# maria-korosteleva/Garment-Pattern-Estimation

Measured on AMD Instinct MI355X. Metric: garments/sec (fwd+bwd) at N=2048 pts, batch 32 per GPU, higher is better.
Workload: dtype f16x3 (fp16 MFMA x3 per product, fp32 accumulate); 1 GPU; BASELINE cfg 2 (cfg 3 per GPU): GarmentFullPattern3D, EdgeConv encoder + LSTM decoders, N=2048, batch 32/GPU, k=16; fp32 storage, fp32-grade arithmetic: edge-GEMM products as 3 fp16 MFMAs on tensor-normalised two-term splits, fp32 accumulate (parity-grade: the exact mode's test bars); global_batch=32, parallelism=dp1, math_mode=f16x3, loss_epoch=0, reserved_cus=0, launch=eager (one Python call per launch), side_stream=True, step=fwd + ComposedPatternLoss + bwd + fused Adam (flat arena)

## Files before the change

garment-pattern-estimation_amd/csrc/gpe_edge_dispatch.h:

```cpp
#pragma once
#include "gpe_rowgemm.h"

#define GPE_EDGE_LAUNCHED 1
#define GPE_EDGE_NOT_MINE 0

static inline bool gpe_edge_width_ok(int c) { return c > 96 && c <= 208; }
static inline int gpe_edge_chunks(int c) { return c <= 160 ? 10 : 13; }
enum { GPE_EDGE_F2 = 0, GPE_EDGE_F3 = 1, GPE_EDGE_B3 = 2, GPE_EDGE_B2 = 3 };
constexpr int gpe_edge_kind(int amode, int emode)
{
    return emode == E_EDGE_FWD ? (amode == A_GATHER ? GPE_EDGE_F2 : GPE_EDGE_F3) : (emode == E_BWD_INPLACE ? GPE_EDGE_B3 : GPE_EDGE_B2);
}
static inline bool gpe_edge_on_menu(const RgParams& p, int amode, int emode)
{
    if (!gpe_edge_width_ok(p.N) || !gpe_edge_width_ok(p.K)) return false;
    if (emode != E_EDGE_FWD && (p.N & 3)) return false;
    if (amode == A_GATHER && (p.K & 3)) return false;
    return !(amode == A_DENSE && (p.a.inner > 0 || (p.a.stride_outer & 3) || p.a.stride_outer < ((p.K + 3) & ~3) || (((uintptr_t)p.a.base) & 15)));
}

int gpe_edge_pseudo_kq(int k);
size_t gpe_edge_pseudo_bytes(long npts, int k, int Cmax);
bool gpe_edge_retile(const RgParams& p_in, int amode, int emode, int stats_nblk, RgParams& p, GpeFold& fold);
int gpe_edge_finish(int rc, const RgParams& p, const GpeFold& fold, hipStream_t s);

int gpe_edge_pc(const RgParams& p, int amode, int emode, int NT, int KCH, int bf16x3, int stats_nblk, hipStream_t s);
int gpe_edge_sr(const RgParams& p, int amode, int emode, int NT, int KCH, int stats_nblk, hipStream_t s);
int gpe_edge_bf16x6(const RgParams& p, int amode, int emode, int NT, int KCH, int stats_nblk, hipStream_t s);
int gpe_edge_f16x3_scales(RgParams& p, long npts, int amode, int emode, int KCH, hipStream_t s);
int gpe_edge_f16x3(const RgParams& p, int amode, int emode, int NT, int KCH, int stats_nblk, hipStream_t s);
int gpe_edge_w8(const RgParams& p, int amode, int emode, int NT, int KCH, int stats_nblk, hipStream_t s);

template <int A, int E> struct GpeEdgeMode { static constexpr int amode = A, emode = E, kind = gpe_edge_kind(A, E); };
template <int AQ_, int BQ_, int KCH_> struct GpeEdgeTile { static constexpr int AQ = AQ_, BQ = BQ_, KCH = KCH_, NT = 4 * AQ_ + BQ_; };

template <class F> static inline int gpe_edge_for_mode(int amode, int emode, F&& f)
{
    if (amode == A_GATHER && emode == E_EDGE_FWD) return f(GpeEdgeMode<A_GATHER, E_EDGE_FWD>{});
    if (amode == A_DENSE && emode == E_EDGE_FWD) return f(GpeEdgeMode<A_DENSE, E_EDGE_FWD>{});
    if (amode == A_DENSE && emode == E_BWD_INPLACE) return f(GpeEdgeMode<A_DENSE, E_BWD_INPLACE>{});
    if (amode == A_DENSE && emode == E_BWD_GATHER) return f(GpeEdgeMode<A_DENSE, E_BWD_GATHER>{});
    return GPE_EINVAL;
}
template <class F> static inline int gpe_edge_for_tile(int NT, int KCH, F&& f)
{
    if (NT == 13 && KCH == 13) return f(GpeEdgeTile<3, 1, 13>{});
    if (NT == 13 && KCH == 10) return f(GpeEdgeTile<3, 1, 10>{});
    if (NT == 10 && KCH == 13) return f(GpeEdgeTile<2, 2, 13>{});
    if (NT == 10 && KCH == 10) return f(GpeEdgeTile<2, 2, 10>{});
    return GPE_EDGE_NOT_MINE;
}
template <class MENU, class F> static inline int gpe_edge_select(int amode, int emode, int NT, int KCH, F&& f)
{
    return gpe_edge_for_mode(amode, emode, [&](auto m) {
        return gpe_edge_for_tile(NT, KCH, [&](auto t) -> int {
            if constexpr (MENU::has(decltype(m)::amode, decltype(m)::emode, decltype(t)::NT, decltype(t)::KCH)) return f(m, t);
            else return GPE_EDGE_NOT_MINE;
        });
    });
}

#define GPE_EDGE_LDS_CAP (160 * 1024)
#define GPE_EDGE_LDS_CAP_STATIC (160 * 1024 - 64)
template <auto KERNEL, int BLOCK, int LDS_CAP> static int gpe_edge_launch(const RgParams& p, int stats_nblk, size_t lds, hipStream_t s)
{
    GPE_ENSURE_MAX_LDS_N(KERNEL, LDS_CAP);
    int gx = gpe_num_cus();
    if (gx > p.num_tiles) gx = p.num_tiles;
    if (stats_nblk > 0 && gx > stats_nblk) gx = stats_nblk;
    hipLaunchKernelGGL(KERNEL, dim3(gx), dim3(BLOCK), lds, s, p, stats_nblk);
    GPE_CHECK_LAUNCH();
    return GPE_EDGE_LAUNCHED;
}
```

garment-pattern-estimation_amd/csrc/gpe_edge_dispatch.hip:

```cpp
#include "gpe_edge_dispatch.h"

static int g_eg_math = 0;
void gpe_edgegemm_set_math(int m) { g_eg_math = m; }

int gpe_edge_pseudo_kq(int k)
{
    int best = 0;
    for (int kq = RG_PB; kq >= RG_PB / RG_NPW; --kq)
        if (k % kq == 0 && (RG_PB / kq) * kq > (best ? (RG_PB / best) * best : 0)) best = kq;
    return best;
}

size_t gpe_edge_pseudo_bytes(long npts, int k, int Cmax)
{
    const int kq = k <= RG_PB ? 0 : gpe_edge_pseudo_kq(k);
    if (!kq) return 0;
    const size_t nps = (size_t)npts * (k / kq), ld = (size_t)((Cmax + 3) & ~3);
    return nps * ld * (2 * sizeof(float) + 2) + 256;
}

static bool edge_pseudo_setup(RgParams& p, bool per_point, int emode, GpeFold& fd)
{
    fd = GpeFold{};
    fd.f = 1;
    if (p.k <= RG_PB) return true;
    if (!per_point) { p.k = 4; return true; }
    const long npts = p.M / p.k;
    const int kq = gpe_edge_pseudo_kq(p.k);
    if (!kq || npts * (p.k / kq) >= (1L << 31) || (p.oldagg & 3) || (p.lddp & 3)) return false;
    fd.f = p.k / kq; fd.kq = kq; fd.npts = npts;
    const long nps = npts * fd.f;
    const bool want_agg = emode == E_EDGE_FWD && p.agg, want_dp = emode == E_BWD_GATHER;
    const size_t agg_f = want_agg ? (size_t)nps * p.oldagg : 0, dp_f = want_dp ? (size_t)nps * p.lddp : 0;
    const size_t bytes = (2 * agg_f + dp_f) * sizeof(float) + 2 * agg_f + 256;
    char* ws = (bytes > 256 && bytes <= p.ws.pseudo_bytes) ? p.ws.pseudo : nullptr;
    if (bytes > 256 && !ws) return false;
    if (want_agg) {
        fd.mx = p.mx; fd.mn = p.mn; fd.amx = p.oamx; fd.amn = p.oamn;
        p.mx = (float*)ws; p.mn = p.mx + agg_f;
        p.oamx = (uint8_t*)(p.mn + agg_f); p.oamn = p.oamx + agg_f;
    }
    if (want_dp) { fd.dp = p.dP; p.dP = (float*)ws; }
    p.k = kq;
    p.pmagic = (unsigned)(((1ull << 32) + fd.f - 1) / fd.f);
    return true;
}

bool gpe_edge_retile(const RgParams& p_in, int amode, int emode, int stats_nblk, RgParams& p, GpeFold& fold)
{
    p = p_in;
    const bool per_point = amode == A_GATHER || emode == E_BWD_GATHER || (emode == E_EDGE_FWD && p.agg);
    if (!edge_pseudo_setup(p, per_point, emode, fold)) return false;
    const int npw = RG_PB / p.k;
    if (per_point && npw > RG_NPW) return false;
    p.R = 4 * npw * p.k;
    p.num_tiles = gpe_cdiv(p.M, p.R);
    p.pin_tpc = 0;
    if ((amode == A_GATHER || emode == E_BWD_GATHER) && p.pin_clouds > 0 && gpe_pin_clouds(p.pin_clouds) &&
        p.pin_clouds % GPE_NXCD == 0) {
        const long rows_per_cloud = p.M / p.pin_clouds;
        const int gx = gpe_num_cus();
        if (rows_per_cloud % p.R == 0 && gx % GPE_NXCD == 0 && gx <= p.num_tiles &&
            (stats_nblk <= 0 || gx <= stats_nblk) && rows_per_cloud / p.R >= gx / GPE_NXCD)
            p.pin_tpc = (int)(rows_per_cloud / p.R);
    }
    return true;
}

int gpe_edge_finish(int rc, const RgParams& p, const GpeFold& fold, hipStream_t s)
{
    if (rc != GPE_EDGE_LAUNCHED) return rc;
    rc = gpe_edge_pseudo_fold(p, fold, s);
    return rc == GPE_OK ? GPE_EDGE_LAUNCHED : rc;
}

int gpe_edgegemm_try(const RgParams& p, int amode, int emode, int stats_nblk, hipStream_t s)
{
    const int math = g_eg_math;
    const bool f16_only = p.out_half || p.lz_g;
    if (!gpe_edge_on_menu(p, amode, emode)) return f16_only ? GPE_EINVAL : GPE_EDGE_NOT_MINE;
    const int NT = gpe_edge_chunks(p.N), KCH = gpe_edge_chunks(p.K);

    RgParams t;
    GpeFold fold;
    const bool tiled = math != 1 && p.k >= 1 && gpe_edge_retile(p, amode, emode, stats_nblk, t, fold);
    int rc;

    if (math == 2 && tiled) {
        rc = gpe_edge_finish(gpe_edge_bf16x6(t, amode, emode, NT, KCH, stats_nblk, s), t, fold, s);
        if (rc != GPE_EDGE_NOT_MINE) return rc;
    }
    if (math == 3 && tiled && p.ws.h3 && p.M >= gpe_h3_min_rows() && !(amode == A_GATHER && !p.user_amax_a && (p.H & 3))) {
        RgParams q = t;
        rc = gpe_edge_f16x3_scales(q, p.M / p.k, amode, emode, KCH, s);
        if (rc != GPE_OK) return rc;
        rc = gpe_edge_w8(q, amode, emode, NT, KCH, stats_nblk, s);
        if (rc == GPE_EDGE_NOT_MINE) rc = gpe_edge_f16x3(q, amode, emode, NT, KCH, stats_nblk, s);
        rc = gpe_edge_finish(rc, q, fold, s);
        if (rc == GPE_EDGE_LAUNCHED && q.amax_out && p.tracked) *p.tracked = 1;
        if (rc != GPE_EDGE_NOT_MINE) return rc;
    }
    if (f16_only) return GPE_EINVAL;

    if (math != 1 && tiled && !(p.dbg & 64)) {
        rc = gpe_edge_finish(gpe_edge_sr(t, amode, emode, NT, KCH, stats_nblk, s), t, fold, s);
        if (rc != GPE_EDGE_NOT_MINE) return rc;
    }
    if (p.R <= 64 && p.k <= 64)
        return gpe_edge_pc(p, amode, emode, NT, KCH, math == 1, stats_nblk, s);
    return GPE_EDGE_NOT_MINE;
}
```

garment-pattern-estimation_amd/csrc/gpe_edgegemm_w8.hip:

```cpp
#include "gpe_edgegemm_w8_kernel.h"

int gpe_w8_select_k5(const RgParams& p, int amode, int emode, int NT, int KCH, int stats_nblk, hipStream_t s);
int gpe_w8_select_k4(const RgParams& p, int amode, int emode, int NT, int KCH, int stats_nblk, hipStream_t s);

static int w8_enabled(int kind)
{
    static int tab[4] = {-1, 0, 0, 0};
    if (tab[0] < 0) {
        const char* e = gpe_dbg_env_str("GPE_W8");
        for (int i = 3; i >= 0; --i) {
            int v = 1;
            if (e && strlen(e) == 4) v = e[i] != '0';
            else if (e && strlen(e) == 1) v = e[0] != '0';
            tab[i] = v;
        }
    }
    return tab[kind];
}

int gpe_edge_w8(const RgParams& p, int amode, int emode, int NT, int KCH, int stats_nblk, hipStream_t s)
{
    if (!((p.k == 16 && p.R == 64 && !p.pmagic) || (p.k == 5 && p.R == 60 && !p.pmagic) || (p.k == 4 && p.R == 64)) || p.M % p.k)
        return GPE_EDGE_NOT_MINE;
    const int kbytes = 2 * ((p.K + 3) & ~3);
    if (kbytes < (KCH == 13 ? 384 : 256)) return GPE_EDGE_NOT_MINE;
    if (p.out_half && !(p.k == 16 && emode == E_EDGE_FWD && amode == A_DENSE && p.agg)) return GPE_EINVAL;
    if (p.lz_g && !(p.k == 16 && emode == E_BWD_INPLACE && amode == A_DENSE)) return GPE_EINVAL;
    if (!w8_enabled(gpe_edge_kind(amode, emode))) return GPE_EDGE_NOT_MINE;
    return p.k == 16 ? w8_select<16>(p, amode, emode, NT, KCH, stats_nblk, s)
           : p.k == 5 ? gpe_w8_select_k5(p, amode, emode, NT, KCH, stats_nblk, s)
                      : gpe_w8_select_k4(p, amode, emode, NT, KCH, stats_nblk, s);
}
```

garment-pattern-estimation_amd/csrc/gpe_edgegemm_w8_kernel.h:

```cpp
#pragma once
#include "gpe_edgegemm_split_kernel.h"
#include <type_traits>

#ifndef W8_SLOT_FENCE
#define W8_SLOT_FENCE 1
#endif
#ifndef W8_B2_SC1
#define W8_B2_SC1 1
#endif
#ifndef W8_BUFSTORE
#define W8_BUFSTORE 11
#endif
__device__ __forceinline__ void w8_pin4(float4& v) { asm volatile("" : "+v"(v.x), "+v"(v.y), "+v"(v.z), "+v"(v.w)); }

template <int NT, int KCH, int AMODE, int EMODE, int AGGT, bool LAZY, int KK = 16>
__global__ __launch_bounds__(512) void gpe_edgegemm_w8_kernel(RgParams p, int stats_nblk)
{
    using SP = SplitF16x2;
    static_assert(KK == 16 || KK == 5 || KK == 4, "neighbourhood sizes with a compile-time row schedule");
    static_assert(!LAZY || KK == 16, "lazy dz3 needs one point per wave");
    constexpr int NPW = 16 / KK;
    constexpr int RW = NPW * KK;
    constexpr int TR = 4 * RW;
    static_assert(NT == 13 || (NT == 10 && KCH == 13), "shapes of the shipped edge MLPs");
    static_assert(KCH == 13 || KCH == 10, "K = 200 / 150");
    static_assert(!LAZY || (AMODE == A_DENSE && EMODE == E_BWD_INPLACE), "lazy dz3: in-place backward");
    static_assert(EMODE != E_BWD_INPLACE || (W8_BUFSTORE & 4) == 0, "the in-place backward loads the rows it overwrites through plain "
                  "pointers: its stores must be plain too (buffer and global accesses are disjoint memory to the compiler)");
    constexpr bool FWD = EMODE == E_EDGE_FWD;
    constexpr bool TRACK = FWD && AGGT != 0;
    constexpr bool OUTH = FWD && AGGT == 2;
    constexpr bool GATHER_ACT = EMODE == E_BWD_GATHER;
    constexpr int KS = (KCH + 1) / 2;
    constexpr bool KTAIL = (KCH & 1) != 0;
    constexpr bool PAIRS = NT == 13;
    constexpr int SL2 = PAIRS ? (KS + 1) / 2 : (KS + 3) / 4;
    constexpr int PPITCH = 16 * x6_pchunks(KCH);
    constexpr int PLANE = RG_BM * PPITCH;
    constexpr int AWORDS = (2 * PLANE) / 4;
    constexpr int LDC = 16 * NT + 4;
    constexpr int NSLOT = 4 * KS;
    constexpr int SPP = (KCH == 13) ? 6 : 4;
    constexpr int NLS = PAIRS ? KS - 1 : 0;
    constexpr int NSCR = PAIRS ? 4 + NLS : 6;
    static_assert(NSCR <= 2 * SPP, "partials do not fit the row");
    constexpr int C0 = (NSLOT >= 28) ? 8 : 6;
    constexpr int I1 = C0 + 4;
    constexpr int C1 = (NSLOT >= 28) ? 22 : 16;
    constexpr int EP0 = NSLOT - 16;
    constexpr int RING = (GATHER_ACT && NPW > 1) ? 6 : 8;

    extern __shared__ __align__(16) float smem[];
    __shared__ unsigned amax_sh[4];
    __shared__ int flag_sh[4];
    float* const Abuf0 = smem;
    float* const Abuf1 = smem + AWORDS;
    float* const Cs = smem + 2 * AWORDS;

    const int tid = threadIdx.x, lane = tid & 63;
    const int wave = __builtin_amdgcn_readfirstlane(tid >> 6);
    const int role = wave >> 2, pt = wave & 3;
    const int j = lane & 15, g = lane >> 4;
    const int g_tail = (g >= 2) ? (g & 1) : g;
    const int rb = RW * pt;
    const int c = lane << 2;
    const bool n_on = c < p.N;
    const int ck = (c < p.K) ? c : ((p.K - 1) & ~3);
    const int cn = n_on ? c : ((p.N - 1) & ~3);

    int rot, sec_tile, sec_slot;
    bool sec_direct, last_on = false, last_direct = false;
    int last_slot = 0;
    if constexpr (PAIRS) {
        rot = role ? pt + SL2 : pt;
        if (rot >= KS) rot -= KS;
        sec_tile = 8 + pt; sec_direct = role == 0; sec_slot = pt;
        last_on = role == 0 || rot >= 4;
        last_direct = wave == 0;
        last_slot = 4 + (role == 0 ? pt - 1 : rot - 1);
    } else {
        rot = 2 * pt;
        sec_tile = 8 + role; sec_direct = pt == 0; sec_slot = 3 * role + pt - 1;
    }

    for (int e = tid; e < 2 * AWORDS; e += 512) smem[e] = 0.f;
    if (tid < 4) flag_sh[tid] = 0;

    float sA, sW, invA, invW;
    SP::scale_of(p.h3_amax_a[0], sA, invA);
    SP::scale_of(p.h3_amax_w[0], sW, invW);

    gpe_u32x4 wP[2][KS], sP[2][SL2], tP[2];
    {
        auto load_frag = [&](int col, int sl) -> X6Frag<SP> {
            const int cc = (col < p.Npad) ? col : p.Npad - 1;
            const int kc = 2 * sl + (g >> 1);
            const bool on = col < p.Npad && kc < KCH;
            const int kcc = kc < KCH ? kc : KCH - 1;
            float4 f0 = ld4(p.wp + (((long)(kcc * 4 + 2 * (g & 1))) * p.Npad + cc) * 4);
            float4 f1 = ld4(p.wp + (((long)(kcc * 4 + 2 * (g & 1) + 1)) * p.Npad + cc) * 4);
            f0 = x6_scale4(f0, sW); f1 = x6_scale4(f1, sW);
            const float4 z = make_float4(0.f, 0.f, 0.f, 0.f);
            return x6_split8<SP>(on ? f0 : z, on ? f1 : z);
        };
#pragma unroll
        for (int i = 0; i < KS; ++i) {
            const int sl = (rot + i >= KS) ? rot + i - KS : rot + i;
            const X6Frag<SP> f = load_frag(16 * wave + j, sl);
            wP[0][i] = f.pl[0]; wP[1][i] = f.pl[1];
        }
#pragma unroll
        for (int i = 0; i < SL2; ++i) {
            const int sl = (rot + i >= KS) ? rot + i - KS : rot + i;
            const bool real = PAIRS ? (role == 0 || i < KS - SL2) : (rot + i < KS);
            const X6Frag<SP> f = load_frag(real ? 16 * sec_tile + j : p.Npad, sl);
            sP[0][i] = f.pl[0]; sP[1][i] = f.pl[1];
        }
        {
            const X6Frag<SP> f = load_frag((PAIRS && last_on) ? 16 * 12 + j : p.Npad, rot);
            tP[0] = f.pl[0]; tP[1] = f.pl[1];
        }
    }

    GpeTileSeq sq = gpe_tile_seq(p.pin_tpc, p.rev, p.pin_clouds, p.num_tiles);

    int vz;
    asm volatile("v_mov_b32 %0, 0" : "=v"(vz));
    int rbl = rb;
#define W8_REFRESH_SCALARS()                                   \
    {                                                          \
        int sz_;                                               \
        asm volatile("s_mov_b32 %0, 0" : "=s"(sz_));           \
        rbl = rb + sz_;                                        \
    }
    auto load_jgv = [&](int tile) -> int {
        const long row0 = (long)tile * TR;
        const int rv = (int)((p.M - row0 < TR) ? (p.M - row0) : TR);
        int r = rbl + ((lane < RW) ? lane : RW - 1);
        r = (r < rv - 1) ? r : rv - 1;
        return p.jg[row0 + r];
    };
    auto prow = [&](long x) -> long { return (KK == 4 && p.pmagic) ? (long)__umulhi((unsigned)x, p.pmagic) : x; };
    auto scr = [&](int row, int s) -> int { return ((s >= SPP ? PLANE + (s - SPP) * 64 : s * 64) + row * PPITCH) >> 2; };

    auto body = [&](auto role_tag) {
        constexpr int ROLE = decltype(role_tag)::value;
        const float4 zero4 = make_float4(0.f, 0.f, 0.f, 0.f);

        float4 v[8];
        constexpr int NPB = NPW > 1 ? 2 : 1;
        float4 pvs[NPB];
#pragma unroll
        for (int q = 0; q < NPB; ++q) pvs[q] = zero4;
        int s_rv = 0, jgv_a = 0, jgv_b = 0;
        float lzs[4] = {0.f, 0.f, 0.f, 0.f}, lznc[4] = {0.f, 0.f, 0.f, 0.f}, lznk[4] = {0.f, 0.f, 0.f, 0.f};
        int lz_sel[4] = {0, 0, 0, 0};
        float lz_won[4] = {0.f, 0.f, 0.f, 0.f};
        float4 lz_gq = zero4;
        uchar4 lz_sx = make_uchar4(0, 0, 0, 0), lz_sn = make_uchar4(0, 0, 0, 0);
        if constexpr (ROLE == 0 && LAZY) {
#pragma unroll
            for (int t = 0; t < 4; ++t) {
                if (ck + t < p.K) {
                    const float k2 = p.lz_coef[2 * p.K + ck + t];
                    lzs[t] = p.lz_coef[ck + t] * sA;
                    lznc[t] = __builtin_fmaf(p.lz_coef[3 * p.K + ck + t], k2, -p.lz_coef[p.K + ck + t]) * sA;
                    lznk[t] = -k2 * sA;
                }
            }
        }
        double stS[4] = {0, 0, 0, 0}, stQ[4] = {0, 0, 0, 0};
        float4 bias4 = zero4, cs4 = zero4, c14 = zero4, k24 = zero4;
        if constexpr (ROLE == 1) {
            {
                if constexpr (FWD) {
                    if (p.bias) {
                        bias4.x = p.bias[cn];
                        if (cn + 1 < p.N) bias4.y = p.bias[cn + 1];
                        if (cn + 2 < p.N) bias4.z = p.bias[cn + 2];
                        if (cn + 3 < p.N) bias4.w = p.bias[cn + 3];
                    }
                } else {
                    cs4 = ld4(p.coef_out + cn); c14 = ld4(p.coef_out + p.N + cn);
                    cs4 = x6_scale4(cs4, invW * invA);
                    k24 = ld4(p.coef_out + 2 * p.N + cn);
                    const float4 mu4 = ld4(p.coef_out + 3 * p.N + cn);
                    c14 = make_float4(__builtin_fmaf(mu4.x, k24.x, -c14.x), __builtin_fmaf(mu4.y, k24.y, -c14.y),
                                      __builtin_fmaf(mu4.z, k24.z, -c14.z), __builtin_fmaf(mu4.w, k24.w, -c14.w));
                    k24 = make_float4(-k24.x, -k24.y, -k24.z, -k24.w);
                }
            }
        }
        const float invAW = invA * invW;
        float amax_run = 0.f;
        float s32[4] = {0.f, 0.f, 0.f, 0.f}, q32[4] = {0.f, 0.f, 0.f, 0.f};
        float vmx[4], vmn[4];
        int imx[4], imn[4];
#pragma unroll
        for (int t = 0; t < 4; ++t) { vmx[t] = -INFINITY; vmn[t] = INFINITY; imx[t] = 0; imn[t] = 0; }
        float4 dp = zero4;
        float4 act[(ROLE == 1 && !FWD) ? RING : 1];
        constexpr int NPE = NPW > 3 ? 2 : NPW;
        float4 pve[NPE];
        long e_ptl = 0;
#pragma unroll
        for (int q = 0; q < NPE; ++q) pve[q] = zero4;
        long e_row0 = 0, e_pt = 0; int e_rv = 0;
        bool epi_on = false;
        __amdgpu_buffer_rsrc_t orsrc = __builtin_amdgcn_make_buffer_rsrc(p.out, 0, 0, 0x00020000);
        float amax_t = 0.f;
        int jgv_e = 0, jgv_cur = 0;

        auto issue_stage_loads = [&](int tile_s, int h) {
            const long row0 = (long)tile_s * TR;
            s_rv = (int)((p.M - row0 < TR) ? (p.M - row0) : TR);
            const int last = s_rv - 1;
            const long pt0 = (long)tile_s * (4 * NPW) + pt * NPW, ptl = (long)tile_s * (4 * NPW) + last / KK;
            const long ptc = pt0 < ptl ? pt0 : ptl;
            if (h == 0) {
                if constexpr (LAZY) {
                    const float* gr = p.lz_g + ptc * p.lz_ldg + ck;
                    const int rem = p.K - 1 - ck;
                    lz_gq = make_float4(gr[0], gr[rem < 1 ? rem : 1], gr[rem < 2 ? rem : 2], gr[rem < 3 ? rem : 3]);
                    lz_sx = *reinterpret_cast<const uchar4*>(p.lz_amx + ptc * p.lz_ldagg + ck);
                    lz_sn = *reinterpret_cast<const uchar4*>(p.lz_amn + ptc * p.lz_ldagg + ck);
                }
            }
            if constexpr (AMODE == A_GATHER) {
                const int pb = (8 * h) / KK;
#pragma unroll
                for (int q = 0; q < NPB; ++q) {
                    const long pg = pt0 + ((pb + q < NPW) ? pb + q : NPW - 1);
                    pvs[q] = ld4(p.pq + (prow(pg < ptl ? pg : ptl) + vz) * p.ldpq + ck);
                }
            }
#pragma unroll
            for (int uu = 0; uu < 8; ++uu) {
                const int u = (8 * h + uu < RW) ? 8 * h + uu : RW - 1;
                int r = rbl + u;
                r = (r < last) ? r : last;
                if constexpr (AMODE == A_GATHER) {
                    const int jj = __builtin_amdgcn_ds_bpermute(u << 2, jgv_a);
                    v[uu] = ld4(p.pq + (long)jj * p.ldpq + p.H + ck);
                } else if constexpr (LAZY) {
                    const uint2 hq = *reinterpret_cast<const uint2*>(reinterpret_cast<const _Float16*>(p.a.base) + (row0 + r) * p.a.stride_outer + ck);
                    v[uu].x = __uint_as_float(hq.x); v[uu].y = __uint_as_float(hq.y);
                } else
                    v[uu] = ld4(p.a.base + (row0 + r) * p.a.stride_outer + ck);
            }
        };
        auto commit_row = [&](float* An, int u) {
            if (u >= RW) return;
            const int r = rbl + u;
            float4 o = v[u & 7];
            if constexpr (AMODE == A_GATHER) {
                const float4 pv = pvs[u / KK - (8 * (u / 8)) / KK];
                o.x = fmaxf(o.x + pv.x, 0.f); o.y = fmaxf(o.y + pv.y, 0.f);
                o.z = fmaxf(o.z + pv.z, 0.f); o.w = fmaxf(o.w + pv.w, 0.f);
            }
            if constexpr (LAZY) {
                const gpe_f32x2 a01 = __builtin_convertvector(__builtin_bit_cast(gpe_f16x2, __float_as_uint(o.x)), gpe_f32x2);
                const gpe_f32x2 a23 = __builtin_convertvector(__builtin_bit_cast(gpe_f16x2, __float_as_uint(o.y)), gpe_f32x2);
                const float av[4] = {a01[0], a01[1], a23[0], a23[1]};
                if (u == 0) {
                    const float gq[4] = {lz_gq.x, lz_gq.y, lz_gq.z, lz_gq.w};
                    const int sx[4] = {lz_sx.x, lz_sx.y, lz_sx.z, lz_sx.w}, sn[4] = {lz_sn.x, lz_sn.y, lz_sn.z, lz_sn.w};
#pragma unroll
                    for (int t = 0; t < 4; ++t) {
                        lz_sel[t] = (lzs[t] >= 0.f) ? sx[t] : sn[t];
                        lz_won[t] = __builtin_fmaf(lzs[t], gq[t], lznc[t]);
                    }
                }
                float dz[4];
#pragma unroll
                for (int t = 0; t < 4; ++t) {
                    const float base = (lz_sel[t] == u) ? lz_won[t] : lznc[t];
                    dz[t] = (av[t] > 0.f) ? __builtin_fmaf(lznk[t], av[t], base) : 0.f;
                }
                o = make_float4(dz[0], dz[1], dz[2], dz[3]);
            }
            if (r >= s_rv) o = zero4;
            unsigned q0[2], q1[2];
            const float sc = LAZY ? 1.f : sA;
            SP::split2(o.x * sc, o.y * sc, q0);
            SP::split2(o.z * sc, o.w * sc, q1);
            char* row = reinterpret_cast<char*>(An) + r * PPITCH + 2 * ck;
            *reinterpret_cast<uint2*>(row) = make_uint2(q0[0], q1[0]);
            *reinterpret_cast<uint2*>(row + PLANE) = make_uint2(q0[1], q1[1]);
        };
        auto wait_folded = [&](int want) {
            int spins = 0;
            while (__hip_atomic_load(&flag_sh[pt], __ATOMIC_ACQUIRE, __HIP_MEMORY_SCOPE_WORKGROUP) < want) {
                __builtin_amdgcn_s_sleep(1);
                if (++spins > (1 << 22)) __builtin_trap();
            }
        };

        auto issue_act_load = [&](int u, int tile_e, int jv) {
            if constexpr (ROLE == 1 && !FWD) {
                const long row0 = (long)tile_e * TR;
                const int rv = (int)((p.M - row0 < TR) ? (p.M - row0) : TR);
                if (u >= RW) u = RW - 1;
                int r = rbl + u;
                r = (r < rv - 1) ? r : rv - 1;
                if constexpr (EMODE == E_BWD_INPLACE) act[u % RING] = ld4(p.out + (row0 + r) * p.ldo + cn);
                else {
                    const int jj = __builtin_amdgcn_ds_bpermute(u << 2, jv);
                    act[u % RING] = ld4(p.pq + (long)jj * p.ldpq + p.H + cn);
                }
            }
        };
        auto begin_epi = [&](int tile_e, bool on) {
            e_row0 = (long)tile_e * TR;
            e_pt = (long)tile_e * (4 * NPW) + pt * NPW;
            e_rv = (int)((p.M - e_row0 < TR) ? (p.M - e_row0) : TR);
            epi_on = on && rbl < e_rv;
            constexpr int ES = OUTH ? 2 : 4;
            orsrc = __builtin_amdgcn_make_buffer_rsrc(reinterpret_cast<char*>(p.out) + e_row0 * p.ldo * ES, 0, RG_BM * p.ldo * ES, 0x00020000);
#pragma unroll
            for (int t = 0; t < 4; ++t) { s32[t] = 0.f; q32[t] = 0.f; vmx[t] = -INFINITY; vmn[t] = INFINITY; imx[t] = 0; imn[t] = 0; }
            dp = zero4;
            amax_t = 0.f;
            if constexpr (GATHER_ACT) {
                const long ptl = (long)tile_e * (4 * NPW) + (e_rv - 1) / KK;
                if constexpr (NPW > NPE) e_ptl = ptl;
#pragma unroll
                for (int q = 0; q < NPE; ++q) pve[q] = ld4(p.pq + (prow(e_pt + q < ptl ? e_pt + q : ptl) + vz) * p.ldpq + cn);
            }
        };
        auto epi_row = [&](int u, float4 z) {
            if (u >= RW) return;
            if constexpr (GATHER_ACT && NPW > NPE) {
                if (u % KK == 0 && u / KK >= 1) {
                    const int q = u / KK;
                    w8_pin4(pve[q % NPE]);
                    if (q + 1 < NPW) {
                        const long pg = e_pt + q + 1;
                        pve[(q + 1) % NPE] = ld4(p.pq + (prow(pg < e_ptl ? pg : e_ptl) + vz) * p.ldpq + cn);
                    }
                }
            }
            w8_pin4(z);
            if constexpr (!FWD) w8_pin4(act[u % RING]);
            if (!epi_on) return;
            const int r = rbl + u;
            if constexpr (KK != 16) {
                if (r >= e_rv) return;
            }
            if constexpr (FWD) {
                const float vv[4] = {fmaxf(__builtin_fmaf(z.x, invAW, bias4.x), 0.f), fmaxf(__builtin_fmaf(z.y, invAW, bias4.y), 0.f),
                                     fmaxf(__builtin_fmaf(z.z, invAW, bias4.z), 0.f), fmaxf(__builtin_fmaf(z.w, invAW, bias4.w), 0.f)};
                if constexpr (!TRACK) amax_t = fmaxf(fmaxf(amax_t, fmaxf(vv[0], vv[1])), fmaxf(vv[2], vv[3]));
                if constexpr (OUTH) {
                    const gpe_f32x2 v01 = {fminf(vv[0], 65504.f), fminf(vv[1], 65504.f)}, v23 = {fminf(vv[2], 65504.f), fminf(vv[3], 65504.f)};
                    const gpe_u32x2 hq = {__builtin_bit_cast(unsigned, __builtin_convertvector(v01, gpe_f16x2)),
                                         __builtin_bit_cast(unsigned, __builtin_convertvector(v23, gpe_f16x2))};
                    if constexpr ((W8_BUFSTORE & 2) != 0)
                        __builtin_amdgcn_raw_buffer_store_b64(hq, orsrc, cn * 2, r * p.ldo * 2, 0);
                    else
                        *reinterpret_cast<uint2*>(reinterpret_cast<_Float16*>(p.out) + (e_row0 + r) * p.ldo + cn) = make_uint2(hq[0], hq[1]);
                } else {
                    const gpe_u32x4 oq = {__float_as_uint(vv[0]), __float_as_uint(vv[1]), __float_as_uint(vv[2]), __float_as_uint(vv[3])};
                    if constexpr ((W8_BUFSTORE & (AMODE == A_GATHER ? 1 : 2)) != 0)
                        __builtin_amdgcn_raw_buffer_store_b128(oq, orsrc, cn * 4, r * p.ldo * 4, AMODE == A_GATHER ? 16 : 0);
                    else
                        st4(p.out + (e_row0 + r) * p.ldo + cn, make_float4(vv[0], vv[1], vv[2], vv[3]));
                }
#pragma unroll
                for (int t = 0; t < 4; ++t) {
                    s32[t] += vv[t];
                    q32[t] = __builtin_fmaf(vv[t], vv[t], q32[t]);
                    if constexpr (TRACK) {
                        if (vv[t] > vmx[t]) { vmx[t] = vv[t]; imx[t] = u % KK; }
                        if (vv[t] < vmn[t]) { vmn[t] = vv[t]; imn[t] = u % KK; }
                    }
                }
            } else {
                float4 av = act[u % RING];
                if constexpr (GATHER_ACT) {
                    const float4 pv = pve[(u / KK) % NPE];
                    av.x = fmaxf(av.x + pv.x, 0.f); av.y = fmaxf(av.y + pv.y, 0.f);
                    av.z = fmaxf(av.z + pv.z, 0.f); av.w = fmaxf(av.w + pv.w, 0.f);
                }
                float4 o;
                o.x = (av.x > 0.f) ? __builtin_fmaf(z.x, cs4.x, __builtin_fmaf(k24.x, av.x, c14.x)) : 0.f;
                o.y = (av.y > 0.f) ? __builtin_fmaf(z.y, cs4.y, __builtin_fmaf(k24.y, av.y, c14.y)) : 0.f;
                o.z = (av.z > 0.f) ? __builtin_fmaf(z.z, cs4.z, __builtin_fmaf(k24.z, av.z, c14.z)) : 0.f;
                o.w = (av.w > 0.f) ? __builtin_fmaf(z.w, cs4.w, __builtin_fmaf(k24.w, av.w, c14.w)) : 0.f;
                const gpe_u32x4 oq = {__float_as_uint(o.x), __float_as_uint(o.y), __float_as_uint(o.z), __float_as_uint(o.w)};
                if constexpr ((W8_BUFSTORE & (EMODE == E_BWD_INPLACE ? 4 : 8)) != 0)
                    __builtin_amdgcn_raw_buffer_store_b128(oq, orsrc, cn * 4, r * p.ldo * 4, (GATHER_ACT && W8_B2_SC1) ? 16 : 0);
                else
                    st4(p.out + (e_row0 + r) * p.ldo + cn, o);
                if constexpr (EMODE == E_BWD_INPLACE)
                    amax_t = fmaxf(fmaxf(amax_t, fmaxf(fabsf(o.x), fabsf(o.y))), fmaxf(fabsf(o.z), fabsf(o.w)));
                dp.x += o.x; dp.y += o.y; dp.z += o.z; dp.w += o.w;
            }
            if (u % KK == KK - 1) {
                if constexpr (TRACK) amax_t = fmaxf(amax_t, fmaxf(fmaxf(vmx[0], vmx[1]), fmaxf(vmx[2], vmx[3])));
                {
                    const long gpt = e_pt + u / KK;
                    if constexpr (TRACK) {
                        const long o = gpt * p.oldagg + cn;
                        st4(p.mx + o, make_float4(vmx[0], vmx[1], vmx[2], vmx[3]));
                        st4(p.mn + o, make_float4(vmn[0], vmn[1], vmn[2], vmn[3]));
                        *reinterpret_cast<uchar4*>(p.oamx + o) = make_uchar4(imx[0], imx[1], imx[2], imx[3]);
                        *reinterpret_cast<uchar4*>(p.oamn + o) = make_uchar4(imn[0], imn[1], imn[2], imn[3]);
                    }
                    if constexpr (GATHER_ACT) st4(p.dP + gpt * p.lddp + cn, dp);
                }
                amax_run = fmaxf(amax_run, amax_t);
                if constexpr (FWD) {
#pragma unroll
                    for (int t = 0; t < 4; ++t) { stS[t] += (double)s32[t]; stQ[t] += (double)q32[t]; }
                }
                if constexpr (NPW > 1) {
#pragma unroll
                    for (int t = 0; t < 4; ++t) { vmx[t] = -INFINITY; vmn[t] = INFINITY; imx[t] = 0; imn[t] = 0; s32[t] = 0.f; q32[t] = 0.f; }
                    dp = zero4;
                }
            }
        };

        int tile = gpe_seq_tile(sq);
        gpe_seq_advance(sq);
        int next = gpe_seq_tile(sq);
        gpe_seq_advance(sq);
        int next2 = gpe_seq_tile(sq);
        if constexpr (ROLE == 0) {
            if (tile < p.num_tiles) {
                if constexpr (AMODE == A_GATHER) jgv_a = load_jgv(tile);
#pragma unroll
                for (int h = 0; h < 2; ++h) {
                    issue_stage_loads(tile, h);
#pragma unroll
                    for (int uu = 0; uu < 8; ++uu) commit_row(Abuf0, 8 * h + uu);
                }
                if constexpr (AMODE == A_GATHER) jgv_b = load_jgv(next < p.num_tiles ? next : tile);
            }
        }
        __syncthreads();

        int buf = 0, prev = -1, iter = 0;
        for (; tile < p.num_tiles; tile = next, next = next2, gpe_seq_advance(sq), next2 = gpe_seq_tile(sq)) {
            W8_REFRESH_SCALARS()
            const float* As = buf ? Abuf1 : Abuf0;
            float* An = buf ? Abuf0 : Abuf1;
            const bool do_epi = prev >= 0;
            const bool do_stage = next < p.num_tiles;
            const int tile_s = do_stage ? next : tile;
            const int tile_e = do_epi ? prev : tile;

            f32x4 acc[4], accS[4], accT[4];
#pragma unroll
            for (int mt = 0; mt < 4; ++mt) {
                acc[mt] = (f32x4){0.f, 0.f, 0.f, 0.f}; accS[mt] = acc[mt]; accT[mt] = acc[mt];
            }
            X6Frag<SP> nf;
            auto read_frag = [&](int i, int mt) {
                const int slr = (rot + i >= KS) ? rot + i - KS : rot + i;
                const int ge = (KTAIL && slr == KS - 1) ? g_tail : g;
                const char* src = reinterpret_cast<const char*>(As) + (16 * mt + j) * PPITCH + 16 * (4 * slr + ge);
                nf.pl[0] = *reinterpret_cast<const gpe_u32x4*>(src);
                nf.pl[1] = *reinterpret_cast<const gpe_u32x4*>(src + PLANE);
            };
            float4 zq = zero4;
            read_frag(0, 0);

#pragma unroll
            for (int i = 0; i < KS; ++i) {
#pragma unroll
                for (int mt = 0; mt < 4; ++mt) {
                    const int q = 4 * i + mt;
                    const X6Frag<SP> af = nf;
                    if (q + 1 < NSLOT) read_frag((q + 1) >> 2, (q + 1) & 3);
                    if constexpr (ROLE == 0) {
                        if (q == 0) {
                            if constexpr (AMODE == A_GATHER) {
                                jgv_a = jgv_b;
                                jgv_b = load_jgv(next2 < p.num_tiles ? next2 : tile);
                            }
                            issue_stage_loads(tile_s, 0);
                        }
                        if (q == C0) wait_folded(iter);
                        if (q >= C0 && q < C0 + 4) { commit_row(An, 2 * (q - C0)); commit_row(An, 2 * (q - C0) + 1); }
                        if (q == I1) issue_stage_loads(tile_s, 1);
                        if (q >= C1 && q < C1 + 4) { commit_row(An, 8 + 2 * (q - C1)); commit_row(An, 9 + 2 * (q - C1)); }
                    } else {
                        if (q == 0) {
                            begin_epi(tile_e, do_epi);
                            if constexpr (GATHER_ACT) { jgv_cur = jgv_e; jgv_e = load_jgv(tile); }
                        }
                        if (q >= EP0 && q - EP0 < RW) {
                            epi_row(q - EP0, zq);
                            if (q - EP0 + RING < RW) issue_act_load(q - EP0 + RING, tile_e, jgv_cur);
                            else issue_act_load((q - EP0) % RING, tile, jgv_e);
                        }
                        if (q + 1 >= EP0 && q + 1 < NSLOT) {
                            const int rr = rbl + ((q + 1 - EP0 < RW) ? q + 1 - EP0 : RW - 1);
                            zq = ld4(&Cs[rr * LDC + cn]);
                        }
                    }
                    acc[mt] = SP::mfma(af.pl[1], wP[0][i], acc[mt]);
                    if (i < SL2) accS[mt] = SP::mfma(af.pl[1], sP[0][i], accS[mt]);
                    if (PAIRS && i == 0) accT[mt] = SP::mfma(af.pl[1], tP[0], accT[mt]);
                    acc[mt] = SP::mfma(af.pl[0], wP[1][i], acc[mt]);
                    if (i < SL2) accS[mt] = SP::mfma(af.pl[0], sP[1][i], accS[mt]);
                    if (PAIRS && i == 0) accT[mt] = SP::mfma(af.pl[0], tP[1], accT[mt]);
                    acc[mt] = SP::mfma(af.pl[0], wP[0][i], acc[mt]);
                    if (i < SL2) accS[mt] = SP::mfma(af.pl[0], sP[0][i], accS[mt]);
                    if (PAIRS && i == 0) accT[mt] = SP::mfma(af.pl[0], tP[0], accT[mt]);
#if W8_SLOT_FENCE
                    __builtin_amdgcn_sched_barrier(0);
#endif
                }
            }
            __syncthreads();
#pragma unroll
            for (int mt = 0; mt < 4; ++mt)
#pragma unroll
                for (int r = 0; r < 4; ++r) Cs[(16 * mt + 4 * g + r) * LDC + 16 * wave + j] = acc[mt][r];
            {
                float* Sc = const_cast<float*>(As);
#pragma unroll
                for (int mt = 0; mt < 4; ++mt)
#pragma unroll
                    for (int r = 0; r < 4; ++r) {
                        const int row = 16 * mt + 4 * g + r;
                        float* dst = sec_direct ? &Cs[row * LDC + 16 * sec_tile + j] : &Sc[scr(row, sec_slot) + j];
                        *dst = accS[mt][r];
                    }
                if constexpr (PAIRS) {
                    if (last_on) {
#pragma unroll
                        for (int mt = 0; mt < 4; ++mt)
#pragma unroll
                            for (int r = 0; r < 4; ++r) {
                                const int row = 16 * mt + 4 * g + r;
                                float* dst = last_direct ? &Cs[row * LDC + 16 * 12 + j] : &Sc[scr(row, last_slot) + j];
                                *dst = accT[mt][r];
                            }
                    }
                }
            }
            __syncthreads();
            if constexpr (ROLE == 1) {
                const int ur = (lane >> 2) < RW ? (lane >> 2) : RW - 1, cq = (lane & 3) << 2;
                const int row = rbl + ur;
                if constexpr (PAIRS) {
#pragma unroll
                    for (int b = 0; b < 4; ++b) {
                        float* cd = &Cs[row * LDC + 16 * (8 + b) + cq];
                        const float4 a0 = ld4(cd), a1 = ld4(&As[scr(row, b) + cq]);
                        st4(cd, make_float4(a0.x + a1.x, a0.y + a1.y, a0.z + a1.z, a0.w + a1.w));
                    }
                    float* cd = &Cs[row * LDC + 16 * 12 + cq];
                    float4 s = ld4(cd);
#pragma unroll
                    for (int l = 0; l < NLS; ++l) {
                        const float4 a1 = ld4(&As[scr(row, 4 + l) + cq]);
                        s.x += a1.x; s.y += a1.y; s.z += a1.z; s.w += a1.w;
                    }
                    st4(cd, s);
                } else {
#pragma unroll
                    for (int b = 0; b < 2; ++b) {
                        float* cd = &Cs[row * LDC + 16 * (8 + b) + cq];
                        float4 s = ld4(cd);
#pragma unroll
                        for (int l = 0; l < 3; ++l) {
                            const float4 a1 = ld4(&As[scr(row, 3 * b + l) + cq]);
                            s.x += a1.x; s.y += a1.y; s.z += a1.z; s.w += a1.w;
                        }
                        st4(cd, s);
                    }
                }
                __hip_atomic_store(&flag_sh[pt], iter + 1, __ATOMIC_RELEASE, __HIP_MEMORY_SCOPE_WORKGROUP);
            }
            prev = tile;
            buf ^= 1;
            ++iter;
        }
        if constexpr (ROLE == 1) {
            {
                W8_REFRESH_SCALARS()
                begin_epi(prev >= 0 ? prev : 0, prev >= 0);
                jgv_cur = jgv_e;
#pragma unroll
                for (int u = 0; u < RW; ++u) {
                    epi_row(u, ld4(&Cs[(rbl + u) * LDC + cn]));
                    if (u + RING < RW) issue_act_load(u + RING, prev >= 0 ? prev : 0, jgv_cur);
                }
            }
            if (p.amax_out && !GATHER_ACT) {
                float m = amax_run;
#pragma unroll
                for (int o = 32; o > 0; o >>= 1) m = fmaxf(m, __shfl_xor(m, o));
                if (lane == 0) amax_sh[pt] = __float_as_uint(m);
            }
        }
        __syncthreads();
        if constexpr (ROLE == 1 && FWD) {
            if (p.stats_part) {
                double* red = reinterpret_cast<double*>(smem);
                if (n_on) {
#pragma unroll
                    for (int t = 0; t < 4; ++t) {
                        red[(pt * 2 + 0) * (16 * NT) + c + t] = stS[t];
                        red[(pt * 2 + 1) * (16 * NT) + c + t] = stQ[t];
                    }
                }
            }
        }
        __syncthreads();
    };
    __syncthreads();
    if (((p.dbg & 1024) || EMODE == E_BWD_GATHER) && role == 1) __builtin_amdgcn_s_setprio(1);
    if ((p.dbg & 2048) && role == 0) __builtin_amdgcn_s_setprio(1);
    if (role == 0) body(std::integral_constant<int, 0>{});
    else body(std::integral_constant<int, 1>{});

    if (p.amax_out && EMODE != E_BWD_GATHER && tid == 0) {
        const unsigned a = amax_sh[0] > amax_sh[1] ? amax_sh[0] : amax_sh[1], b = amax_sh[2] > amax_sh[3] ? amax_sh[2] : amax_sh[3];
        atomicMax(p.amax_out, a > b ? a : b);
    }
    if (FWD && p.stats_part && tid < p.N) {
        const double* red = reinterpret_cast<const double*>(smem);
        constexpr int NC = 16 * NT;
        const double ss = (red[0 * NC + tid] + red[2 * NC + tid]) + (red[4 * NC + tid] + red[6 * NC + tid]);
        const double qq = (red[1 * NC + tid] + red[3 * NC + tid]) + (red[5 * NC + tid] + red[7 * NC + tid]);
        for (int b = blockIdx.x; b < stats_nblk; b += gridDim.x) {
            double* dst = p.stats_part + (size_t)b * 2 * p.N;
            dst[tid] = (b == (int)blockIdx.x) ? ss : 0.0;
            dst[p.N + tid] = (b == (int)blockIdx.x) ? qq : 0.0;
        }
    }
#undef W8_REFRESH_SCALARS
}

template <int NT, int KCH, int AMODE, int EMODE, int AGGT, bool LAZY, int KK = 16>
static int w8_launch(const RgParams& p, int stats_nblk, hipStream_t s)
{
    constexpr int LDC = 16 * NT + 4;
    constexpr int AWORDS = (2 * RG_BM * 16 * x6_pchunks(KCH)) / 4;
    const size_t lds = (size_t)(2 * AWORDS + RG_BM * LDC) * sizeof(float);
    return gpe_edge_launch<gpe_edgegemm_w8_kernel<NT, KCH, AMODE, EMODE, AGGT, LAZY, KK>, 512, GPE_EDGE_LDS_CAP_STATIC>(p, stats_nblk, lds, s);
}

struct W8Menu {
    static constexpr bool has(int amode, int emode, int NT, int KCH)
    {
        const int kind = gpe_edge_kind(amode, emode);
        return kind == GPE_EDGE_F3 ? (NT == 10 && KCH == 13) : kind == GPE_EDGE_B3 ? (NT == 13 && KCH == 10) : (NT == 13 && KCH == 13);
    }
};
int gpe_w8_launch_f3(const RgParams& p, int stats_nblk, hipStream_t s);
int gpe_w8_launch_b3(const RgParams& p, int stats_nblk, hipStream_t s);

template <int KK>
static int w8_select(const RgParams& p, int amode, int emode, int NT, int KCH, int stats_nblk, hipStream_t s)
{
    return gpe_edge_select<W8Menu>(amode, emode, NT, KCH, [&](auto m, auto t) -> int {
        using M = decltype(m);
        using T = decltype(t);
        if ((M::kind == GPE_EDGE_F2 && p.agg) || (M::kind == GPE_EDGE_F3 && !p.agg)) return GPE_EDGE_NOT_MINE;
        if constexpr (KK == 16 && M::kind == GPE_EDGE_F3) return gpe_w8_launch_f3(p, stats_nblk, s);
        else if constexpr (KK == 16 && M::kind == GPE_EDGE_B3) return gpe_w8_launch_b3(p, stats_nblk, s);
        else return w8_launch<T::NT, T::KCH, M::amode, M::emode, M::kind == GPE_EDGE_F2 ? 0 : M::kind == GPE_EDGE_F3 ? 1 : -1, false, KK>(p, stats_nblk, s);
    });
}
```

garment-pattern-estimation_amd/csrc/gpe_rowgemm.h:

```cpp
#pragma once
#include "gpe_device.h"

#define RG_BM 64
#define RG_KSLAB 256
#define RG_PB 16
#define RG_NPW 4

enum { A_DENSE = 0, A_GATHER = 1 };
enum { E_LINEAR = 0, E_EDGE_FWD = 1, E_BWD_INPLACE = 2, E_BWD_GATHER = 3 };

struct RgParams {
    long M;
    int N, K;
    int R;
    int num_tiles;
    GpeRows a;
    const float* pq; int ldpq; int H;
    const int32_t* jg; int k; double rcp_k;
    const float* wp; int Npad;
    const float* bias;
    GpeRows addend;
    float* y; long y_so, y_si; int y_inner; int act;
    float* out; int ldo;
    double* stats_part;
    int agg; float* mx; float* mn; uint8_t* oamx; uint8_t* oamn; int oldagg;
    const float* coef_out;
    float* dP; int lddp;
    int dbg;
    int pin_tpc;
    int rev;
    int pin_clouds;
    unsigned pmagic;
    float* dummy;
    const unsigned* h3_amax_a;
    const unsigned* h3_amax_w;
    unsigned* amax_out;
    const float* lz_g; int lz_ldg;
    const uint8_t* lz_amx; const uint8_t* lz_amn; int lz_ldagg;
    const float* lz_coef;
    int out_half;
    int w_ready;
    const unsigned* user_amax_a;
    unsigned* user_amax_out;
    GpeEdgeWs ws;
    int* tracked;
};

struct GpeFold {
    int f, kq;
    long npts;
    float *mx, *mn, *dp;
    uint8_t *amx, *amn;
};
int gpe_edge_pseudo_fold(const RgParams& p, const GpeFold& fd, hipStream_t s);

__device__ __forceinline__ float4 ld4(const float* p) { return *reinterpret_cast<const float4*>(p); }
__device__ __forceinline__ void st4(float* p, float4 v) { *reinterpret_cast<float4*>(p) = v; }
__device__ __forceinline__ void st4_stream(float* p, float4 v)
{
    const f32x4 vv = {v.x, v.y, v.z, v.w};
    asm volatile("global_store_dwordx4 %0, %1, off sc1" : : "v"(p), "v"(vv) : "memory");
}

__device__ __forceinline__ float rg_pin_agpr(float x)
{
    float a;
    asm volatile("v_accvgpr_write_b32 %0, %1" : "=a"(a) : "v"(x));
    return a;
}
__device__ __forceinline__ float4 rg_pin_agpr4(const float4 v)
{
    return make_float4(rg_pin_agpr(v.x), rg_pin_agpr(v.y), rg_pin_agpr(v.z), rg_pin_agpr(v.w));
}

__device__ __forceinline__ float4 rg_sel4(const float4 a0, const float4 a1, const float4 a2, const float4 a3, int idx)
{
    float4 r = a0;
    r.x = (idx == 1) ? a1.x : r.x; r.y = (idx == 1) ? a1.y : r.y; r.z = (idx == 1) ? a1.z : r.z; r.w = (idx == 1) ? a1.w : r.w;
    r.x = (idx == 2) ? a2.x : r.x; r.y = (idx == 2) ? a2.y : r.y; r.z = (idx == 2) ? a2.z : r.z; r.w = (idx == 2) ? a2.w : r.w;
    r.x = (idx == 3) ? a3.x : r.x; r.y = (idx == 3) ? a3.y : r.y; r.z = (idx == 3) ? a3.z : r.z; r.w = (idx == 3) ? a3.w : r.w;
    return r;
}

__device__ __forceinline__ long rg_prow(int x, unsigned magic) { return magic ? (long)__umulhi((unsigned)x, magic) : (long)x; }
template <bool PSEUDO>
__device__ __forceinline__ long rg_prow(int x, unsigned magic) { return PSEUDO ? (long)__umulhi((unsigned)x, magic) : (long)x; }

__device__ __forceinline__ float4 ld4_guard(const float* p, int nvalid, bool vec)
{
    if (nvalid >= 4 && vec) return ld4(p);
    float4 v = make_float4(0.f, 0.f, 0.f, 0.f);
    if (nvalid > 0) v.x = p[0];
    if (nvalid > 1) v.y = p[1];
    if (nvalid > 2) v.z = p[2];
    if (nvalid > 3) v.w = p[3];
    return v;
}

template <int EMODE>
__device__ __forceinline__ void rg_epilogue(const RgParams& p, float* Cs, int ldc, long row0, int rv, int n0,
                                            int ncols, double& st_sum, double& st_sq)
{
    const int tid = threadIdx.x;
    const int c = (tid & 63) << 2;
    const int rw = tid >> 6;
    if (EMODE == E_LINEAR) {
        if (c < ncols) {
            const int nvalid = ncols - c;
            for (int r = rw; r < rv; r += 4) {
                const long gr = row0 + r;
                const float4 v = ld4(&Cs[r * ldc + c]);
                float o[4] = {v.x, v.y, v.z, v.w};
                const float* ad = nullptr;
                if (p.addend.base) ad = gpe_row_ptr(p.addend, gr) + n0 + c;
                float* dst;
                if (p.y_inner <= 0) dst = p.y + gr * p.y_so + n0 + c;
                else { long oo = gr / p.y_inner; dst = p.y + oo * p.y_so + (gr - oo * p.y_inner) * p.y_si + n0 + c; }
#pragma unroll
                for (int t = 0; t < 4; ++t) {
                    if (t < nvalid) {
                        float x = o[t];
                        if (p.bias) x += p.bias[n0 + c + t];
                        if (ad) x += ad[t];
                        if (p.act == 1) x = fmaxf(x, 0.f);
                        o[t] = x;
                    }
                }
                if (nvalid >= 4 && gpe_aligned16(dst)) st4(dst, make_float4(o[0], o[1], o[2], o[3]));
                else {
#pragma unroll
                    for (int t = 0; t < 4; ++t) if (t < nvalid) dst[t] = o[t];
                }
            }
        }
    } else if (EMODE == E_EDGE_FWD) {
        if (tid < ncols) {
            const float bz = p.bias ? p.bias[n0 + tid] : 0.f;
            for (int r = 0; r < rv; ++r) {
                const float v = fmaxf(Cs[r * ldc + tid] + bz, 0.f);
                Cs[r * ldc + tid] = v;
                st_sum += (double)v;
                st_sq += (double)v * (double)v;
            }
        }
        __syncthreads();
        if (c < ncols)
            for (int r = rw; r < rv; r += 4) st4(p.out + (row0 + r) * p.ldo + n0 + c, ld4(&Cs[r * ldc + c]));
        if (p.agg) {
            if (tid < ncols) {
                const int pts = rv / p.k;
                const long pt0 = (long)gpe_udiv((unsigned)row0, (unsigned)p.k, p.rcp_k);
                for (int pt = 0; pt < pts; ++pt) {
                    const float* col = &Cs[(pt * p.k) * ldc + tid];
                    float vmx = col[0], vmn = col[0];
                    int imx = 0, imn = 0;
                    for (int s = 1; s < p.k; ++s) {
                        const float v = col[s * ldc];
                        if (v > vmx) { vmx = v; imx = s; }
                        if (v < vmn) { vmn = v; imn = s; }
                    }
                    const long o = (pt0 + pt) * p.oldagg + n0 + tid;
                    p.mx[o] = vmx; p.mn[o] = vmn;
                    p.oamx[o] = (uint8_t)imx; p.oamn[o] = (uint8_t)imn;
                }
            }
        }
    } else {
        if (c < ncols) {
            const int nvalid = ncols - c;
            float cs_[4], c1_[4], k2_[4], mu_[4];
#pragma unroll
            for (int t = 0; t < 4; ++t) {
                const int cc = n0 + c + (t < nvalid ? t : 0);
                cs_[t] = p.coef_out[cc]; c1_[t] = p.coef_out[p.N + cc];
                k2_[t] = p.coef_out[2 * p.N + cc]; mu_[t] = p.coef_out[3 * p.N + cc];
            }
            for (int r = rw; r < rv; r += 4) {
                const long gr = row0 + r;
                const float4 u4 = ld4(&Cs[r * ldc + c]);
                float* dst = p.out + gr * p.ldo + n0 + c;
                float4 act;
                if (EMODE == E_BWD_INPLACE) {
                    act = ld4(dst);
                } else {
                    const long i = (long)gpe_udiv((unsigned)gr, (unsigned)p.k, p.rcp_k);
                    const long jj = p.jg[gr];
                    const float4 a = ld4(p.pq + i * p.ldpq + n0 + c);
                    const float4 b = ld4(p.pq + jj * p.ldpq + p.H + n0 + c);
                    act = make_float4(fmaxf(a.x + b.x, 0.f), fmaxf(a.y + b.y, 0.f), fmaxf(a.z + b.z, 0.f),
                                      fmaxf(a.w + b.w, 0.f));
                }
                const float uv[4] = {u4.x, u4.y, u4.z, u4.w};
                const float av[4] = {act.x, act.y, act.z, act.w};
                float o[4];
#pragma unroll
                for (int t = 0; t < 4; ++t) {
                    o[t] = 0.f;
                    if (t < nvalid && av[t] > 0.f) o[t] = uv[t] * cs_[t] - c1_[t] - (av[t] - mu_[t]) * k2_[t];
                }
                const float4 o4 = make_float4(o[0], o[1], o[2], o[3]);
                st4(dst, o4);
                if (EMODE == E_BWD_GATHER) st4(&Cs[r * ldc + c], o4);
            }
        }
        if (EMODE == E_BWD_GATHER) {
            __syncthreads();
            if (tid < ncols) {
                const int pts = rv / p.k;
                const long pt0 = (long)gpe_udiv((unsigned)row0, (unsigned)p.k, p.rcp_k);
                for (int pt = 0; pt < pts; ++pt) {
                    const float* col = &Cs[(pt * p.k) * ldc + tid];
                    float s = 0.f;
                    for (int t = 0; t < p.k; ++t) s += col[t * ldc];
                    p.dP[(pt0 + pt) * p.lddp + n0 + tid] = s;
                }
            }
        }
    }
}
```

garment-pattern-estimation_amd/csrc/gpe_rowgemm.hip:

```cpp
#include "gpe_common.h"

#include "gpe_edge_dispatch.h"

template <int AMODE>
__device__ __forceinline__ void rg_build_a(const RgParams& p, float* As, int lda, long row0, int rv, int ks,
                                           int kslab, int kp)
{
    const int tid = threadIdx.x;
    const int c = (tid & 63) << 2;
    if (c >= kp) return;
    const int nvalid = kslab - c;
    for (int r = tid >> 6; r < RG_BM; r += 4) {
        float4 v = make_float4(0.f, 0.f, 0.f, 0.f);
        if (r < rv && nvalid > 0) {
            const long gr = row0 + r;
            if (AMODE == A_DENSE) {
                const float* src = gpe_row_ptr(p.a, gr) + ks + c;
                v = ld4_guard(src, nvalid, gpe_aligned16(src));
            } else {
                const long i = (long)gpe_udiv((unsigned)gr, (unsigned)p.k, p.rcp_k);
                const long j = p.jg[gr];
                const float* pp = p.pq + i * p.ldpq + ks + c;
                const float* qq = p.pq + j * p.ldpq + p.H + ks + c;
                const float4 a = ld4_guard(pp, nvalid, gpe_aligned16(pp));
// ... 143 lines not shown
    const int need = gpe_cdiv(N, 16);
    const int opts[5] = {4, 7, 10, 13, 16};
    for (int i = 0; i < 5; ++i) if (opts[i] >= need) return opts[i];
    return -1;
}

int gpe_smallgemm_linear(const RgParams& r, hipStream_t s);
int gpe_edgegemm_try(const RgParams& p, int amode, int emode, int stats_nblk, hipStream_t s);

void gpe_edgegemm_set_math(int m);
void gpe_redgemm_set_math(int m);

int gpe_gemm_x6_linear(const GpeRows& a, const float* wp, int Npad, int Kq, const float* bias, const GpeRows& addend, float* y,
                       long y_so, long y_si, int y_inner, long M, int N, int K, int act, hipStream_t s);
extern "C" long gpe_packed_size(int N, int K);
static int g_gpe_dbg = 0;
extern "C" int gpe_debug_set(int flags) { g_gpe_dbg = flags; return 0; }
extern "C" int gpe_debug_get(void) { return g_gpe_dbg; }
static int g_gpe_math = 0;
extern "C" int gpe_edge_lazy_dz3_ok(int B, int N, int k, int F, int Cprev);
extern "C" int gpe_math_get(void) { return g_gpe_math; }
extern "C" int gpe_math_set(int mode)
{
    if (mode < 0 || mode > 4) return GPE_EINVAL;
    const int prev = g_gpe_math;
    g_gpe_math = mode;
    gpe_edgegemm_set_math(mode == 4 ? 3 : mode == 3 ? 2 : (mode != 0 ? 1 : 0));
    gpe_redgemm_set_math(mode == 1 ? 1 : mode == 4 ? 2 : 0);
    return prev;
}

#define GPE_STATS_BLOCKS 512
extern "C" int gpe_stats_blocks(void) { return GPE_STATS_BLOCKS; }

extern "C" long gpe_edge_ws_bytes(int B, int N, int k, int ldmax)
{
    if (B <= 0 || N <= 0 || k <= 0 || ldmax <= 0) return GPE_EINVAL;
    return (long)(GPE_WS_DUMMY_BYTES + GPE_WS_H3_BYTES) + (long)gpe_edge_pseudo_bytes((long)B * N, k, ldmax);
}
static long g_h3_min_rows = GPE_H3_MIN_ROWS_DEFAULT;
long gpe_h3_min_rows() { return g_h3_min_rows; }
extern "C" long gpe_f16x3_min_rows(void) { return g_h3_min_rows; }
extern "C" long gpe_f16x3_min_rows_set(long rows)
{
    if (rows < 0) return GPE_EINVAL;
    const long prev = g_h3_min_rows;
    g_h3_min_rows = rows;
    return prev;
}
extern "C" int gpe_edge_pq_amax(const float* pq, int ldpq, int H, long rows, uint32_t* amax, void* ws, long ws_bytes,
                                void* stream)
{
    const GpeEdgeWs w = gpe_edge_ws(ws, ws_bytes);
    if (!pq || !amax || !w.h3 || rows <= 0 || H <= 0 || (H & 3) || (ldpq & 3) || ldpq < 2 * H) return GPE_EINVAL;
    return gpe_h3_pq_passes(amax, reinterpret_cast<float*>(w.h3 + 2), pq, rows, H, ldpq, (hipStream_t)stream);
}
extern "C" int gpe_absmax(const float* x, int ldx, long rows, int cols, uint32_t* amax, void* stream)
{
    if (!x || !amax || rows < 0 || cols <= 0 || ldx < cols || (ldx & 3) || (((uintptr_t)x) & 15)) return GPE_EINVAL;
    return gpe_h3_absmax(amax, x, rows, cols, ldx, (hipStream_t)stream);
}

#define RG_SMALLK 8
__global__ __launch_bounds__(256) void gpe_linear_smallk_kernel(RgParams p)
{
    const int lane = threadIdx.x & 63;
    const int wave = __builtin_amdgcn_readfirstlane(threadIdx.x >> 6);
    const int c = (blockIdx.y * 64 + lane) << 2;
    if (c >= p.N) return;
    float w[RG_SMALLK][4];
    float b4[4] = {0.f, 0.f, 0.f, 0.f};
#pragma unroll
    for (int k = 0; k < RG_SMALLK; ++k) {
#pragma unroll
        for (int t = 0; t < 4; ++t) {
            w[k][t] = (k < p.K) ? p.wp[((long)(((k >> 4) << 2) + ((k >> 2) & 3)) * p.Npad + c + t) * 4 + (k & 3)] : 0.f;
        }
    }
    if (p.bias) {
#pragma unroll
        for (int t = 0; t < 4; ++t) b4[t] = p.bias[c + t];
    }
    const long nw = (long)gridDim.x * 4;
    for (long r = (long)blockIdx.x * 4 + wave; r < p.M; r += nw) {
        const float* ar = gpe_row_ptr(p.a, r);
        float av[RG_SMALLK];
#pragma unroll
        for (int k = 0; k < RG_SMALLK; ++k) av[k] = ar[k < p.K ? k : 0];
        float o[4] = {b4[0], b4[1], b4[2], b4[3]};
#pragma unroll
        for (int k = 0; k < RG_SMALLK; ++k) {
            if (k < p.K) {
#pragma unroll
                for (int t = 0; t < 4; ++t) o[t] = __builtin_fmaf(av[k], w[k][t], o[t]);
            }
        }
        if (p.addend.base) {
            const float4 ad = ld4(gpe_row_ptr(p.addend, r) + c);
            o[0] += ad.x; o[1] += ad.y; o[2] += ad.z; o[3] += ad.w;
        }
        if (p.act == 1) {
#pragma unroll
            for (int t = 0; t < 4; ++t) o[t] = fmaxf(o[t], 0.f);
        }
        float* dst;
        if (p.y_inner <= 0) dst = p.y + r * p.y_so + c;
        else { const long oo = r / p.y_inner; dst = p.y + oo * p.y_so + (r - oo * p.y_inner) * p.y_si + c; }
        st4(dst, make_float4(o[0], o[1], o[2], o[3]));
    }
}

static bool rg_rows_aligned16(const float* base, long so, long si, int inner)
{
    return !(((uintptr_t)base) & 15) && !(so & 3) && (inner <= 0 || !(si & 3));
}

extern "C" int gpe_linear(const float* a, long a_so, long a_si, int a_inner, const float* wp, const float* bias,
                          const float* addend, long ad_so, long ad_si, int ad_inner, float* y, long y_so,
                          long y_si, int y_inner, int M, int N, int K, int act, void* stream)
{
    if (!a || !wp || !y || M < 0 || N <= 0 || K <= 0 || (act != 0 && act != 1)) return GPE_EINVAL;
    if (M == 0) return GPE_OK;
    RgParams p = {};
    p.M = M; p.N = N; p.K = K; p.R = RG_BM; p.num_tiles = gpe_cdiv(M, RG_BM);
    p.a = GpeRows{a, a_so, a_si, a_inner};
    p.wp = wp; p.Npad = gpe_round_up(N, 16); p.bias = bias;
    p.addend = GpeRows{addend, ad_so, ad_si, ad_inner};
    p.y = y; p.y_so = y_so; p.y_si = y_si; p.y_inner = y_inner; p.act = act;
    if (g_gpe_math == 4 && !(g_gpe_dbg & 16384)) {
        const int rc = gpe_gemm_x6_linear(p.a, wp, p.Npad, (int)(gpe_packed_size(N, K) / p.Npad / 4), bias, p.addend, y, y_so, y_si, y_inner, M, N, K,
                                          act, (hipStream_t)stream);
        if (rc != 0) return rc < 0 ? rc : GPE_OK;
    }
    if (K <= RG_SMALLK && !(N & 3) && M >= 4096 && rg_rows_aligned16(y, y_so, y_si, y_inner) &&
        (!addend || rg_rows_aligned16(addend, ad_so, ad_si, ad_inner))) {
        long gx = gpe_cdiv(M, 4 * 8);
        if (gx > 4096) gx = 4096;
        hipLaunchKernelGGL(gpe_linear_smallk_kernel, dim3((unsigned)gx, gpe_cdiv(N, 256)), dim3(256), 0, (hipStream_t)stream, p);
        GPE_CHECK_LAUNCH();
        return GPE_OK;
    }
    if ((long)p.num_tiles * gpe_cdiv(N, 208) < 128) return gpe_smallgemm_linear(p, (hipStream_t)stream);
    int NT = 4;
    const int opts[5] = {16, 13, 10, 7, 4};
    for (int i = 0; i < 5; ++i) {
        const int nblk = gpe_cdiv(N, 16 * opts[i]);
        if ((long)nblk * p.num_tiles >= 256 || opts[i] == 4) { NT = opts[i]; break; }
    }
    const int single = rg_pick_nt_single(N);
    if (single > 0 && single < NT) NT = single;
    if (N > 256) {
        int best = NT, best_pad = gpe_cdiv(N, 16 * NT) * 16 * NT;
        const int wide[3] = {16, 13, 10};
        for (int i = 0; i < 3; ++i) {
            const int pad = gpe_cdiv(N, 16 * wide[i]) * 16 * wide[i];
            if (pad < best_pad && (long)gpe_cdiv(N, 16 * wide[i]) * p.num_tiles >= 256) { best = wide[i]; best_pad = pad; }
        }
        NT = best;
    }
    dim3 grid(p.num_tiles, gpe_cdiv(N, 16 * NT));
    return rg_dispatch_nt<A_DENSE, E_LINEAR>(NT, p, grid, (hipStream_t)stream);
}

extern "C" int gpe_edge_lazy_dz3_ok(int B, int N, int k, int F, int Cprev)
{
    static const int dbg_off = gpe_dbg_env("GPE_LAZY_DZ3", 1) == 0;
    if (dbg_off || (g_gpe_dbg & 512) || g_gpe_math != 4 || k != 16 || B <= 0 || N <= 0) return 0;
    if (!gpe_edge_width_ok(F) || !gpe_edge_width_ok(Cprev) || (Cprev & 3)) return 0;
    if (gpe_cdiv(Cprev, 16) != 13 || (gpe_cdiv(F, 16) != 10 && gpe_cdiv(F, 16) != 13)) return 0;
    const long rows = (long)B * N * k;
    return rows >= gpe_h3_min_rows() && rows < (1L << 31) && rows / 32 >= 4L * 2 * gpe_num_cus();
}

__global__ __launch_bounds__(256) void gpe_dz3_bound_kernel(const unsigned* __restrict__ amax_sg, const float* __restrict__ coef, int F,
                                                            const unsigned* __restrict__ amax_a3, unsigned* __restrict__ out)
{
    __shared__ float red[4];
    const int lane = threadIdx.x & 63, wave = threadIdx.x >> 6;
    const float a3 = __uint_as_float(amax_a3[0]) * 1.001f;
    float tail = 0.f;
    for (int c = threadIdx.x; c < F; c += 256)
        tail = fmaxf(tail, fabsf(coef[F + c]) + (a3 + fabsf(coef[3 * F + c])) * fabsf(coef[2 * F + c]));
#pragma unroll
    for (int o = 32; o > 0; o >>= 1) tail = fmaxf(tail, __shfl_xor(tail, o));
    if (lane == 0) red[wave] = tail;
    __syncthreads();
    if (threadIdx.x == 0) {
        tail = fmaxf(fmaxf(red[0], red[1]), fmaxf(red[2], red[3]));
        const float b = (__uint_as_float(amax_sg[0]) + tail) * 1.000001f;
        out[0] = __float_as_uint(b) & 0x7fffffffu;
    }
}
extern "C" int gpe_edge_dz3_bound(const uint32_t* amax_sg, const float* coef, int F, const uint32_t* amax_a3, uint32_t* amax_out,
                                  void* stream)
{
    if (!amax_sg || !coef || !amax_a3 || !amax_out || F <= 0) return GPE_EINVAL;
    hipLaunchKernelGGL(gpe_dz3_bound_kernel, dim3(1), dim3(256), 0, (hipStream_t)stream, amax_sg, coef, F, amax_a3, amax_out);
    GPE_CHECK_LAUNCH();
    return GPE_OK;
}

extern "C" int gpe_edge_mlp_fwd(int a_mode, const float* pq, int ldpq, const int32_t* jg, const float* a_in,
                                int lda, int B, int N, int k, int Cin, int Cout, const float* wp,
                                const float* bias, float* out, int ldo, double* stats_part, int agg, float* mx,
                                float* mn, uint8_t* amx, uint8_t* amn, int ldagg, const uint32_t* amax_a,
                                uint32_t* amax_out, void* ws, long ws_bytes, int out_half, void* stream)
{
    if (!wp || !out || B <= 0 || N <= 0 || k <= 0 || k > 64 || Cin <= 0 || Cout <= 0 || (ldo & 3) || ldo < Cout)
        return GPE_EINVAL;
    const int w_ready = (out_half >> 1) & 1;
    out_half &= 1;
    if (out_half && (a_mode != 1 || !agg || !gpe_edge_lazy_dz3_ok(B, N, k, Cout, Cin))) return GPE_EINVAL;
    if (a_mode == 0 && (!pq || !jg || (ldpq & 3) || (Cin & 3) || Cin > RG_KSLAB)) return GPE_EINVAL;
    if (a_mode == 1 && (!a_in || lda < Cin)) return GPE_EINVAL;
    if (agg && (!mx || !mn || !amx || !amn || ldagg < Cout)) return GPE_EINVAL;
    {
        const size_t E_ = (size_t)B * N * k, P_ = (size_t)B * N, ob = E_ * ldo * (out_half ? 2 : 4);
        if (gpe_overlap(out, ob, a_mode == 1 ? a_in : nullptr, E_ * lda * 4) || gpe_overlap(out, ob, a_mode == 0 ? pq : nullptr, P_ * ldpq * 4) ||
            gpe_overlap(out, ob, agg ? mx : nullptr, P_ * ldagg * 4) || gpe_overlap(out, ob, agg ? mn : nullptr, P_ * ldagg * 4))
            return GPE_EINVAL;
    }
    const int NT = (Cout > 256) ? 13 : rg_pick_nt_single(Cout);
    if (NT < 0) return GPE_EINVAL;
    const int ny = gpe_cdiv(Cout, 16 * NT);
    if (ny > 1 && a_mode == 0) return GPE_EINVAL;
    RgParams p = {};
    p.M = (long)B * N * k; p.N = Cout; p.K = Cin;
    p.R = (RG_BM / k) * k; p.num_tiles = gpe_cdiv(p.M, p.R);
    p.a = GpeRows{a_in, lda, 0, 0};
    p.pq = pq; p.ldpq = ldpq; p.H = Cin; p.jg = jg; p.k = k; p.rcp_k = 1.0 / k;
    p.wp = wp; p.Npad = gpe_round_up(Cout, 16); p.bias = bias;
    p.out = out; p.ldo = ldo; p.stats_part = stats_part;
    p.agg = agg; p.mx = mx; p.mn = mn; p.oamx = amx; p.oamn = amn; p.oldagg = ldagg;
    p.dbg = g_gpe_dbg; p.pin_clouds = B;
    p.user_amax_a = amax_a; p.user_amax_out = amax_out; p.ws = gpe_edge_ws(ws, ws_bytes);
    p.out_half = out_half;
    p.w_ready = w_ready;
    p.rev = gpe_walk_rev(a_mode == 1);
    int tracked = 0;
    p.tracked = &tracked;
    int rc = gpe_edgegemm_try(p, a_mode == 0 ? A_GATHER : A_DENSE, E_EDGE_FWD,
                              stats_part ? GPE_STATS_BLOCKS : 0, (hipStream_t)stream);
    if (rc == 0) {
        dim3 grid(GPE_STATS_BLOCKS, ny);
        rc = (a_mode == 0) ? rg_dispatch_nt<A_GATHER, E_EDGE_FWD>(NT, p, grid, (hipStream_t)stream)
                           : rg_dispatch_nt<A_DENSE, E_EDGE_FWD>(NT, p, grid, (hipStream_t)stream);
    } else
        rc = rc == 1 ? GPE_OK : rc;
    if (rc == GPE_OK && out_half && !tracked) return GPE_EINVAL;
    if (rc == GPE_OK && amax_out && !tracked) rc = gpe_h3_absmax(amax_out, out, p.M, Cout, ldo, (hipStream_t)stream);
    return rc;
}

extern "C" int gpe_edge_mlp_bwd(const float* a, int lda, int act_mode, const float* pq, int ldpq,
                                const int32_t* jg, int B, int N, int k, int Cin, int Cout, const float* wp,
                                const float* coef_out, float* dz_out, int ldo, float* dP, int lddp,
                                const uint32_t* amax_a, uint32_t* amax_out, void* ws, long ws_bytes, const float* lz_g, int lz_ldg,
                                const uint8_t* lz_amx, const uint8_t* lz_amn, int lz_ldagg, const float* lz_coef, void* stream)
{
    if (!a || !wp || !coef_out || !dz_out || B <= 0 || N <= 0 || k <= 0 || k > 64 || Cin <= 0 || Cout <= 0 ||
        (ldo & 3) || ldo < Cout || lda < Cin)
        return GPE_EINVAL;
    if (act_mode == 1 && (!pq || !jg || !dP || (ldpq & 3) || (Cout & 3) || Cout > 256)) return GPE_EINVAL;
    {
        const size_t E_ = (size_t)B * N * k, P_ = (size_t)B * N, ob = E_ * ldo * 4;
        const bool in_place = act_mode == 1 && !lz_g && (const void*)a == (const void*)dz_out && lda == ldo;
        if ((!in_place && gpe_overlap(dz_out, ob, a, E_ * lda * (lz_g ? 2 : 4))) || gpe_overlap(dz_out, ob, act_mode == 1 ? pq : nullptr, P_ * ldpq * 4) ||
            gpe_overlap(dz_out, ob, act_mode == 1 ? dP : nullptr, P_ * lddp * 4))
            return GPE_EINVAL;
    }
    const int NT = (Cout > 256) ? 13 : rg_pick_nt_single(Cout);
    if (NT < 0) return GPE_EINVAL;
    const int ny = gpe_cdiv(Cout, 16 * NT);
    RgParams p = {};
    p.M = (long)B * N * k; p.N = Cout; p.K = Cin;
    p.R = (RG_BM / k) * k; p.num_tiles = gpe_cdiv(p.M, p.R);
    p.a = GpeRows{a, lda, 0, 0};
    p.pq = pq; p.ldpq = ldpq; p.H = Cout; p.jg = jg; p.k = k; p.rcp_k = 1.0 / k;
    p.wp = wp; p.Npad = gpe_round_up(Cout, 16);
    p.out = dz_out; p.ldo = ldo; p.coef_out = coef_out; p.dP = dP; p.lddp = lddp;
    hipStream_t s = (hipStream_t)stream;
    p.dbg = g_gpe_dbg; p.pin_clouds = B;
    p.user_amax_a = amax_a; p.user_amax_out = amax_out; p.ws = gpe_edge_ws(ws, ws_bytes);
    p.rev = gpe_walk_rev(1);
    if (lz_g) {
        if (!lz_amx || !lz_amn || !lz_coef || lz_ldg < Cin || (lz_ldagg & 3) || lz_ldagg < ((Cin + 3) & ~3) || act_mode != 0 || !amax_a ||
            !gpe_edge_lazy_dz3_ok(B, N, k, Cin, Cout) || !p.ws.h3)
            return GPE_EINVAL;
        p.lz_g = lz_g; p.lz_ldg = lz_ldg; p.lz_amx = lz_amx; p.lz_amn = lz_amn; p.lz_ldagg = lz_ldagg; p.lz_coef = lz_coef;
    }
    int tracked = 0;
    p.tracked = &tracked;
    int rc = gpe_edgegemm_try(p, A_DENSE, act_mode == 1 ? E_BWD_GATHER : E_BWD_INPLACE, 0, s);
    if (lz_g && rc != 1) return rc < 0 ? rc : GPE_EINVAL;
    if (rc == 0) {
        dim3 grid(p.num_tiles < 2048 ? p.num_tiles : 2048, ny);
        rc = (act_mode == 1) ? rg_dispatch_nt<A_DENSE, E_BWD_GATHER>(NT, p, grid, s)
                             : rg_dispatch_nt<A_DENSE, E_BWD_INPLACE>(NT, p, grid, s);
    } else
        rc = rc == 1 ? GPE_OK : rc;
    if (rc == GPE_OK && amax_out && !tracked) rc = gpe_h3_absmax(amax_out, dz_out, p.M, Cout, ldo, s);
    return rc;
}
```

garment-pattern-estimation_amd/ops.py:

```python
import contextlib
import math
import os
import warnings
import weakref

import numpy as np
import torch

from . import _lib as L
from . import streams

F32 = torch.float32


def _dev_check(t):
    if not t.is_cuda:
        raise RuntimeError('gpe ops need tensors on the MI355X (got a %s tensor); there is no CPU path' % t.device)
    if t.dtype != F32:
        raise RuntimeError('gpe ops are fp32 (got %s)' % t.dtype)


def _rows2d(t):
    assert t.dim() == 2 and (t.shape[1] == 1 or t.stride(1) == 1), (t.shape, t.stride())
    return (t, t.stride(0), 0, 0)


def _rows3d(t):
    assert t.dim() == 3 and (t.shape[2] == 1 or t.stride(2) == 1), (t.shape, t.stride())
    return (t, t.stride(0), t.stride(1), t.shape[1])


def round_up(a, b):
    return (a + b - 1) // b * b


_WS = {}


def _workspace(nbytes, device):
    key = streams.stream_key(device)
    buf = _WS.get(key)
    if buf is None or buf.numel() < nbytes:
        buf = torch.empty(max(int(nbytes), 1 << 20), device=torch.device('cuda', key[0]), dtype=torch.uint8)
        _WS[key] = buf
    return buf


_EDGE_WS_BYTES = {}


def edge_workspace(B, N, k, ldmax, device):
    key = (B, N, k, ldmax)
    n = _EDGE_WS_BYTES.get(key)
    if n is None:
        n = L.query('gpe_edge_ws_bytes', B, N, k, ldmax)
        if n < 0:
            raise RuntimeError('gpe_edge_ws_bytes failed with code %d' % n)
        _EDGE_WS_BYTES[key] = n
    return _workspace(n, device), n


def f16x3_words(n, rows, device):
    if L.get_math() != 'f16x3' or rows < L.query('gpe_f16x3_min_rows'):
        return None
    return torch.zeros(n, device=device, dtype=torch.int32)


def _word(words, i):
    return None if words is None else words[i:i + 1]


_TICKETS = {}


def _ticket(device):
    key = streams.stream_key(device)
    t = _TICKETS.get(key)
    if t is None:
        t = _TICKETS[key] = torch.zeros(1, device=torch.device('cuda', key[0]), dtype=torch.int32)
    return t


def pack_fold(W, bias, stats, ews, ews_n, clear_word):
    N, K = W.shape
    wp = torch.empty(L.query('gpe_packed_size', N, K), device=W.device, dtype=F32)
    bf = torch.empty(N, device=W.device, dtype=F32)
    L.call('gpe_pack_fold', W, W.stride(0), N, K, stats[2], stats[3], bias, wp, bf, ews, ews_n if ews is not None else 0, clear_word,
           _ticket(W.device) if ews is not None else None)
    return wp, bf


SIDE_GRADS = not (os.environ.get('GPE_DEBUG') == '1' and os.environ.get('GPE_SIDE_GRADS') == '0')
SIDE_MIN_EDGES = 1 << 17
SIDE_PQ = not (os.environ.get('GPE_DEBUG') == '1' and os.environ.get('GPE_SIDE_PQ') == '0')
_LAST_EDGES = [0]


def _side_ok(edges):
    return bool(SIDE_GRADS and edges >= SIDE_MIN_EDGES and not torch.cuda.is_current_stream_capturing())


def side_grads(params, tensors):
    if params and _side_ok(_LAST_EDGES[0]) and all(_SINK.get(p.data_ptr()) is not None and _SINK[p.data_ptr()][0]() is not None for p in params):
        return streams.lane(params[0].device.index).fork(tensors, leaf=True)
    return contextlib.nullcontext(False)


WEIGHTS_EPOCH = 0
_PACKS = {}

K_PLAIN, K_TRANS, K_GATES, K_PQ, K_PQT, K_VADD, K_BPQ, K_GRUB = 0, 1, 2, 3, 4, 5, 6, 7
K_GATES_H3, K_AMAX, K_TRANS_H3 = 8, 9, 10
_JOB = np.dtype([('w', '<u8'), ('w2', '<u8'), ('out', '<u8'), ('total', '<i8'), ('first_block', '<i8'),
                 ('ldw', '<i4'), ('N', '<i4'), ('K', '<i4'), ('kind', '<i4'), ('Npad', '<i4'), ('aux', '<i4')])
assert _JOB.itemsize == 64




def bump_weights_epoch():
    global WEIGHTS_EPOCH
    WEIGHTS_EPOCH += 1


class PackPlan:

    def __init__(self):
        self.specs = []
        self.outs = []
        self.table = None
        self.blocks = 0
        self.vers = None
        self.epoch = -1
        self.home = None
        self.keys = []
        self.frozen = False
        self.h3_current = False
        self._stream = None
        self._keys_box = box = []
        me = weakref.ref(self)
        weakref.finalize(self, lambda: [_PACKS.pop(k, None) for k in box if (_PACKS.get(k) or (None,))[0] is me])
        self._me = me

    def _add(self, p, kind, N, K, aux=0, p2=None, out_numel=None):
        self.specs.append((p, p2, kind, N, K, aux, out_numel))

    def add_linear(self, w, fwd=True, bwd=True):
        if fwd:
            self._add(w, K_PLAIN, w.shape[0], w.shape[1])
        if bwd:
            self._add(w, K_TRANS, w.shape[1], w.shape[0])

    def add_gates(self, w, H, G=4):
        self._add(w, K_GATES, G * H, w.shape[1], aux=H)
        self._add(w, K_GATES_H3, G * H, w.shape[1], aux=H)
        if G == 4:
            self._add(w, K_TRANS_H3, w.shape[1], G * H)

    def add_edge_first(self, w1, b1):
        H, C2 = w1.shape
        C = C2 // 2
        self._add(w1, K_PQ, 2 * H, C, aux=H)
        self._add(w1, K_PQT, C, 2 * H, aux=H)
        self._add(b1, K_BPQ, 2 * H, 0, aux=H, out_numel=2 * H)

    def add_bias_sum(self, b_ih, b_hh):
        self._add(b_ih, K_VADD, b_ih.numel(), 0, p2=b_hh, out_numel=b_ih.numel())

    def add_gru_bias(self, b_ih, b_hh, H):
        self._add(b_ih, K_GRUB, b_ih.numel(), 0, aux=2 * H, p2=b_hh, out_numel=b_ih.numel())

    def _versions(self):
        return [p._version + (p2._version if p2 is not None else 0) for p, p2, *_ in self.specs]

    def _build(self):
        for k in self.keys:
            if (_PACKS.get(k) or (None,))[0] is self._me:
                _PACKS.pop(k, None)
        self.keys, self.outs = [], []
        del self._keys_box[:]
        dev = self.specs[0][0].device
        tab = np.zeros(len(self.specs), dtype=_JOB)
        blk = 0
        h3 = [i for i, sp in enumerate(self.specs) if sp[2] in (K_GATES_H3, K_TRANS_H3)]
        mats = []
        for i in h3:
            if all(self.specs[i][0] is not self.specs[j][0] for j in mats):
                mats.append(i)
        self.words = torch.zeros(max(len(mats), 1), device=dev, dtype=torch.int32)
        pre = np.zeros(len(mats), dtype=_JOB)
        pblk = 0
        for wi, i in enumerate(mats):
            p = self.specs[i][0]
            n_el = p.numel()
            pre[wi] = (p.data_ptr(), 0, self.words[wi:wi + 1].data_ptr(), n_el, pblk, p.stride(0), p.shape[0], p.shape[1], K_AMAX, 0, 0)
            pblk += L.query('gpe_pack_job_blocks', K_AMAX, n_el, 0, 0)
        self.pre_blocks = pblk
        self.pre_table = torch.from_numpy(pre.view(np.uint8).copy()).to(dev) if h3 else None
        self.word_of = {}
        for i, (p, p2, kind, N, K, aux, out_numel) in enumerate(self.specs):
            w2 = p2.data_ptr() if p2 is not None else 0
            if kind in (K_VADD, K_BPQ, K_GRUB):
                total, npad = out_numel, 0
            elif kind == K_GATES:
                npad = 16 * (N // aux) * ((aux + 15) // 16)
                total = npad * round_up(K, 16)
            elif kind in (K_GATES_H3, K_TRANS_H3):
                npad = 16 * (N // aux) * ((aux + 15) // 16) if kind == K_GATES_H3 else round_up(N, 16)
                total = L.query('gpe_packed_planes_size', npad, K)
                wi = [j for j, m_ in enumerate(mats) if self.specs[m_][0] is p][0]
                word = self.words[wi:wi + 1]
                w2 = word.data_ptr()
                self.word_of[(p.data_ptr(), kind)] = word
            else:
                npad = round_up(N, 16)
                total = L.query('gpe_packed_size', N, K)
            out = torch.empty(total, device=dev, dtype=F32)
            self.outs.append(out)
            tab[i] = (p.data_ptr(), w2, out.data_ptr(), total, blk,
                      p.stride(0) if p.dim() == 2 else 0, N, K, kind, npad, aux)
            blk += L.query('gpe_pack_job_blocks', kind, total, npad, K)
            key = (p.data_ptr(), kind)
            _PACKS[key] = (self._me, out, i)
            self.keys.append(key)
            self._keys_box.append(key)
        self.blocks = blk
        self.table = torch.from_numpy(tab.view(np.uint8).copy()).to(dev)
        keep = [i for i in range(len(self.specs)) if i not in h3]
        tab2 = tab[keep].copy()
        blk2 = 0
        for j in range(len(keep)):
            tab2[j]['first_block'] = blk2
            blk2 += L.query('gpe_pack_job_blocks', int(tab2[j]['kind']), int(tab2[j]['total']), int(tab2[j]['Npad']), int(tab2[j]['K']))
        self.table_noh3 = torch.from_numpy(tab2.view(np.uint8).copy()).to(dev) if h3 else self.table
        self.blocks_noh3, self.n_noh3 = (blk2, len(keep)) if h3 else (blk, len(self.specs))
        self.home = self._home()

    def _home(self):
        return tuple((p.data_ptr(), p2.data_ptr() if p2 is not None else 0, p.device) for p, p2, *_ in self.specs)

    def refresh(self):
        if not self.specs:
            return
        vers = self._versions()
        if self.specs[0][0].is_cuda:
            st = torch.cuda.current_stream(self.specs[0][0].device)
            if self._stream is not None and st != self._stream:
                st.wait_stream(self._stream)
            self._stream = st
        if self.table is None or self.home != self._home():
            self._build()
        elif (self.frozen and self.vers == vers and self.epoch == WEIGHTS_EPOCH and
              self.h3_current == (self.pre_table is not None and L.get_math() == 'f16x3')):
            return
        self.h3_current = self.pre_table is not None and L.get_math() == 'f16x3'

        def launches():
            if self.h3_current:
                self.words.zero_()
                L.call('gpe_pack_multi', self.pre_table, self.pre_table.numel() // 64, self.pre_blocks)
                L.call('gpe_pack_multi', self.table, len(self.specs), self.blocks)
            else:
                L.call('gpe_pack_multi', self.table_noh3, self.n_noh3, self.blocks_noh3)

        launches()
        self.vers, self.epoch = vers, WEIGHTS_EPOCH


def _planned(t, kind, t2=None):
    hit = _PACKS.get((t.data_ptr(), kind))
    if hit is None:
        return None
    plan, out, i = hit
    plan = plan()
    if plan is None or plan.vers is None or plan.epoch != WEIGHTS_EPOCH:
        return None
    if plan.vers[i] != t._version + (t2._version if t2 is not None else 0):
        return None
    return out


_SINK = {}


def _gbuf(param, shape=None):
    hit = _SINK.get(param.data_ptr())
    if hit is not None and hit[0]() is not None:
        return hit[1]
    return torch.empty(param.shape if shape is None else shape, device=param.device, dtype=F32)


def _gret(param, buf):
    hit = _SINK.get(param.data_ptr())
    arena = hit[0]() if hit is not None else None
    if arena is None:
        return buf
    arena.mark_written(param)
    return None


def pack_weight(w, transpose=False, col_scale=None):
    _dev_check(w)
    assert w.dim() == 2 and w.stride(1) == 1
    if col_scale is None:
        hit = _planned(w, K_TRANS if transpose else K_PLAIN)
        if hit is not None:
            return hit
    N, K = (w.shape[1], w.shape[0]) if transpose else (w.shape[0], w.shape[1])
    wp = torch.empty(L.query('gpe_packed_size', N, K), device=w.device, dtype=F32)
    L.call('gpe_pack_weight', w, w.stride(0), N, K, int(transpose), col_scale, wp)
    return wp


def pack_gates(w, H, G=4):
    hit = _planned(w, K_GATES)
    if hit is not None:
        return hit
    wp = torch.empty(L.query('gpe_packed_ngates_size', H, G, w.shape[1]), device=w.device, dtype=F32)
    L.call('gpe_pack_weight_ngates', w, w.stride(0), H, G, w.shape[1], wp)
    return wp


def planned_planes(w, kind):
    hit = _PACKS.get((w.data_ptr(), kind))
    if hit is None:
        return None, None
    plan = hit[0]()
    out = _planned(w, kind)
    if plan is None or out is None or not plan.h3_current:
        return None, None
    return out, plan.word_of.get((w.data_ptr(), kind))


def bias_sum(b_ih, b_hh):
    hit = _planned(b_ih, K_VADD, b_hh)
    if hit is not None:
        return hit
    out = torch.empty_like(b_ih)
    L.call('gpe_add', b_ih, b_hh, out, b_ih.numel())
    return out


def gru_bias(b_ih, b_hh, H):
    hit = _planned(b_ih, K_GRUB, b_hh)
    if hit is not None:
        return hit
    out = b_ih.detach().clone()
    L.call('gpe_add', b_ih, b_hh, out, 2 * H)
    return out


def _ptr_array(tensors):
    import ctypes
    return (ctypes.c_void_p * len(tensors))(*[t.data_ptr() if t is not None else None for t in tensors])


def edge_first_operands(W1, b1):
    H, C = W1.shape[0], W1.shape[1] // 2
    a, b, c = _planned(W1, K_PQ), _planned(W1, K_PQT), _planned(b1, K_BPQ)
    if a is not None and b is not None and c is not None:
        return a, b, c
    wpq = torch.empty(2 * H, C, device=W1.device, dtype=F32)
    bpq = torch.empty(2 * H, device=W1.device, dtype=F32)
    L.call('gpe_w1_split', W1, W1.stride(0), b1, H, C, wpq, C, bpq)
    return pack_weight(wpq), pack_weight(wpq, transpose=True), bpq


def fold_bias(w, bias, t):
    out = torch.empty(w.shape[0], device=w.device, dtype=F32)
    L.call('gpe_fold_bias', w, w.stride(0), w.shape[0], w.shape[1], bias, t, out)
    return out


def linear_raw(a_desc, wp, bias, M, N, K, y_desc, act=0, addend_desc=None):
    ad = addend_desc if addend_desc is not None else (None, 0, 0, 0)
    L.call('gpe_linear', a_desc[0], a_desc[1], a_desc[2], a_desc[3], wp, bias,
           ad[0], ad[1], ad[2], ad[3], y_desc[0], y_desc[1], y_desc[2], y_desc[3], M, N, K, act)


def redgemm_raw(u_desc, v_desc, rows, Mg, Ng, want_colsum=True, accumulate_into=None, v_shift=None, out=None):
    dev = u_desc[0].device
    if accumulate_into is not None:
        G, cs = accumulate_into
    elif out is not None:
        G, cs = out
    else:
        G = torch.empty(Mg, Ng, device=dev, dtype=F32)
        cs = torch.empty(Mg, device=dev, dtype=F32) if want_colsum else None
    acc = int(accumulate_into is not None)
    for n0 in range(0, Ng, 256):
        nb = min(256, Ng - n0)
        ws = torch.empty(L.query('gpe_redgemm_ws', Mg, nb), device=dev, dtype=F32)
        L.call('gpe_redgemm', u_desc[0], u_desc[1], u_desc[2], u_desc[3],
               v_desc[0][..., n0:], v_desc[1], v_desc[2], v_desc[3], None if v_shift is None else v_shift[n0:],
               rows, Mg, nb, G[:, n0:], G.stride(0), cs if n0 == 0 else None, ws, acc)
    return G, cs


def knn(x, B, N, k, want_global=False, order=None, want_order=False):
    _dev_check(x)
    idx = torch.empty(B, N, k, device=x.device, dtype=torch.int32)
    jg = torch.empty(B, N, k, device=x.device, dtype=torch.int32) if want_global else None
    oo = torch.empty(B, N, device=x.device, dtype=torch.int32) if want_order else None
    if order is not None:
        assert order.dtype == torch.int32 and order.shape == (B, N) and order.is_contiguous() and order.device == x.device
    nws = L.query('gpe_knn_ws_bytes', B, N, x.shape[1], k)
    L.call('gpe_knn', x, B, N, x.shape[1], x.stride(0), k, idx, jg, order, oo, _workspace(nws, x.device), nws)
    out = (idx, jg) if want_global else (idx,)
    if want_order:
        out = out + (oo,)
    return out if len(out) > 1 else out[0]


def knn_reverse(idx):
    B, N, k = idx.shape
    off = torch.empty(B, N + 1, device=idx.device, dtype=torch.int32)
    edge = torch.empty(B, N * k, device=idx.device, dtype=torch.int32)
    L.call('gpe_knn_reverse', idx, B, N, k, off, edge)
    return off, edge


def bn_finalize(part, nblk, C, count, gamma, beta, eps, momentum, rm, rv, nbt):
    stats = torch.empty(4, C, device=gamma.device, dtype=F32)
    L.call('gpe_bn_finalize', part, nblk, C, float(count), gamma, beta, float(eps), float(momentum), rm, rv, nbt,
           stats)
    return stats


def bn_from_running(rm, rv, gamma, beta, eps):
    C = gamma.shape[0]
    stats = torch.empty(4, C, device=gamma.device, dtype=F32)
    L.call('gpe_bn_from_running', rm, rv, C, gamma, beta, float(eps), stats)
    return stats


def bn_bwd_coef(part, nblk, stats, C, count, gamma=None, beta=None, training=True):
    dev = stats.device
    coef = torch.empty(4, C, device=dev, dtype=F32)
    dg = _gbuf(gamma) if gamma is not None else torch.empty(C, device=dev, dtype=F32)
    db = _gbuf(beta) if beta is not None else torch.empty(C, device=dev, dtype=F32)
    L.call('gpe_bn_bwd_coef', part, nblk, stats, C, float(count), coef, dg, db)
    if not training:
        coef[1:3].zero_()
    return coef, dg, db


class LinearFn(torch.autograd.Function):

    @staticmethod
    def forward(ctx, x, weight, bias):
        _dev_check(x)
        K = x.shape[-1]
        M = x.numel() // K
        N = weight.shape[0]
        y = torch.empty(M, N, device=x.device, dtype=F32)
        linear_raw(_rows3d(x) if x.dim() == 3 else _rows2d(x), pack_weight(weight), bias, M, N, K, _rows2d(y))
        ctx.save_for_backward(x, weight, bias)
        return y

    @staticmethod
    def backward(ctx, gy):
        x, weight, bias = ctx.saved_tensors
        gy = gy.contiguous()
        K = x.shape[-1]
        M = x.numel() // K
        N = weight.shape[0]
        xd = _rows3d(x) if x.dim() == 3 else _rows2d(x)
        gx = gw = gb = None
        if ctx.needs_input_grad[0]:
            gx = torch.empty(*x.shape, device=x.device, dtype=F32)
            linear_raw(_rows2d(gy), pack_weight(weight, transpose=True), None, M, K, N, (gx, K, 0, 0))
        if ctx.needs_input_grad[1] or bias is not None:
            with side_grads([weight, bias] if bias is not None else [], [gy, x]):
                gw = _gbuf(weight)
                gb = _gbuf(bias) if bias is not None else torch.empty(N, device=x.device, dtype=F32)
                redgemm_raw(_rows2d(gy), xd, M, N, K, out=(gw, gb))
                gw = _gret(weight, gw)
                gb = _gret(bias, gb) if bias is not None else None
        return gx, gw, gb


def linear(x, weight, bias=None):
    return LinearFn.apply(x, weight, bias)


POOL_MODES = {'mean': 0, 'max': 1, 'add': 2}


class SegmentMeanFn(torch.autograd.Function):

    @staticmethod
    def forward(ctx, x, B, N):
        _dev_check(x)
        C = x.shape[1]
        y = torch.empty(B, C, device=x.device, dtype=F32)
        L.call('gpe_segment_mean_fwd', x, x.stride(0), B, N, C, y, C)
        ctx.dims = (B, N, C)
        return y

    @staticmethod
    def backward(ctx, gy):
        B, N, C = ctx.dims
        gy = gy.contiguous()
        gx = torch.empty(B * N, C, device=gy.device, dtype=F32)
        L.call('gpe_segment_mean_bwd', gy, C, B, N, C, gx, C, 0)
        return gx, None, None


class SegmentPoolFn(torch.autograd.Function):

    @staticmethod
    def forward(ctx, x, B, N, mode):
        _dev_check(x)
        C = x.shape[1]
        y = torch.empty(B, C, device=x.device, dtype=F32)
        arg = torch.empty(B, C, device=x.device, dtype=torch.int32) if mode == 1 else None
        L.call('gpe_segment_pool_fwd', x, x.stride(0), B, N, C, mode, y, C, arg)
        ctx.dims = (B, N, C, mode)
        ctx.arg = arg
        return y

    @staticmethod
    def backward(ctx, gy):
        B, N, C, mode = ctx.dims
        gy = gy.contiguous()
        gx = torch.empty(B * N, C, device=gy.device, dtype=F32)
        L.call('gpe_segment_pool_bwd', gy, C, ctx.arg, B, N, C, mode, gx, C)
        return gx, None, None, None


def segment_mean(x, B, N):
    return SegmentMeanFn.apply(x, B, N)


def segment_max(x, B, N):
    return SegmentPoolFn.apply(x, B, N, 1)


def segment_add(x, B, N):
    return SegmentPoolFn.apply(x, B, N, 2)


segment_mean.pool_mode, segment_max.pool_mode, segment_add.pool_mode = 0, 1, 2


_HALF_ACT_GUARD = 'fallback'
CAPTURE = None
HOST_DRAWN = None


def set_half_act_guard(mode):
    global _HALF_ACT_GUARD
    if mode not in ('fallback', 'strict', 'off'):
        raise ValueError("half-activation guard mode must be 'fallback', 'strict' or 'off'")
    prev, _HALF_ACT_GUARD = _HALF_ACT_GUARD, mode
    return prev


if os.environ.get('GPE_HALF_ACT_GUARD'):
    set_half_act_guard(os.environ['GPE_HALF_ACT_GUARD'])


class HalfActGuard:
    LIMIT = 65504.0

    def __init__(self):
        self.disabled = False
        self.last_amax = None
        self._pending = None

    def __getstate__(self):
        return {'disabled': self.disabled, 'last_amax': self.last_amax, '_pending': None}

    def __deepcopy__(self, memo):
        g = HalfActGuard()
        g.disabled, g.last_amax = self.disabled, self.last_amax
        return g

    @staticmethod
    def _value(host):
        return float(np.array([int(host[0])], dtype=np.int32).view(np.float32)[0])

    def _trip(self, v):
        self.disabled = True
        warnings.warn('f16x3: the aggregated EdgeConv activation reached %.3g (fp16 storage clamps at 65504): this layer keeps it '
                      'in fp32 and forms dz3 eagerly from now on (gpe_amd.ops.set_half_act_guard)' % v, RuntimeWarning, stacklevel=3)

    def allow(self):
        if _HALF_ACT_GUARD == 'off':
            return True
        if CAPTURE is not None:
            return not self.disabled
        if self._pending is not None and self._pending[1].query():
            v = self._value(self._pending[0])
            self._pending = None
            self.last_amax = v
            if not v < self.LIMIT:
                self._trip(v)
        return not self.disabled

    def watch(self, word):
        if _HALF_ACT_GUARD == 'off':
            return True
        if CAPTURE is not None:
            CAPTURE.guards.append((self, word))
            return True
        if _HALF_ACT_GUARD == 'strict':
            v = self._value(word.cpu())
            self.last_amax = v
            if not v < self.LIMIT:
                self._trip(v)
                return False
            return True
        if self._pending is not None:
            self.allow()
            if self._pending is not None:
                return True
        host = torch.empty(1, dtype=torch.int32, pin_memory=True)
        host.copy_(word, non_blocking=True)
        ev = torch.cuda.Event()
        ev.record()
        self._pending = (host, ev)
        return True


class EdgeConvFn(torch.autograd.Function):

    @staticmethod
    def forward(ctx, x, B, N, k, training, eps, momentum, nb, aggr, guard, order, *tensors):
        _dev_check(x)
        ctx.set_materialize_grads(False)
        dev = x.device
        BN, C = x.shape
        assert BN == B * N
        params, bufs = tensors[:4 * nb], tensors[4 * nb:]
        Ws = [params[4 * l] for l in range(nb)]
        widths = [w.shape[0] for w in Ws]
        H0 = widths[0]
        assert Ws[0].shape[1] == 2 * C
        if H0 % 4 or H0 > 256:
            raise ValueError('EdgeConvFn (the fused P|Q path) needs a first-block width that is a multiple of 4 and <= 256 '
                             '(got %d): use ops.edge_conv_general' % H0)
        E = BN * k
        _LAST_EDGES[0] = E
        nblk = L.query('gpe_stats_blocks')
        wpq_p, _, bpq = edge_first_operands(Ws[0], params[1])
        ews, ews_n = edge_workspace(B, N, k, max(round_up(widths[-1], 4), 2 * H0), dev)
        words = f16x3_words(2 * nb + 1, E, dev)
        fork = SIDE_PQ and _side_ok(E)
        if fork:
            lane = streams.lane(dev.index)
            with lane.fork([x, words]):
                PQ = torch.empty(BN, 2 * H0, device=dev, dtype=F32)
                linear_raw(_rows2d(x), wpq_p, bpq, BN, 2 * H0, C, _rows2d(PQ))
                if words is not None:
                    sws, sws_n = edge_workspace(B, N, k, max(round_up(widths[-1], 4), 2 * H0), dev)
                    L.call('gpe_edge_pq_amax', PQ, 2 * H0, H0, BN, _word(words, 0), sws, sws_n)
            idx, jg, order_out = knn(x, B, N, k, want_global=True, order=order, want_order=True)
            lane.wait(made=[PQ])
        else:
            idx, jg, order_out = knn(x, B, N, k, want_global=True, order=order, want_order=True)
            PQ = torch.empty(BN, 2 * H0, device=dev, dtype=F32)
            linear_raw(_rows2d(x), wpq_p, bpq, BN, 2 * H0, C, _rows2d(PQ))
            if words is not None:
                L.call('gpe_edge_pq_amax', PQ, 2 * H0, H0, BN, _word(words, 0), ews, ews_n)

        def stats_of(part, l):
            g, be = params[4 * l + 2], params[4 * l + 3]
            rm, rv, nbt = bufs[3 * l: 3 * l + 3]
            if training:
                return bn_finalize(part, nblk, widths[l], E, g, be, eps, momentum, rm, rv, nbt)
            return bn_from_running(rm, rv, g, be, eps)

        part = torch.empty(nblk, 2, H0, device=dev, dtype=torch.float64) if training else None
        if training:
            L.call('gpe_edge_gather_stats', PQ, 2 * H0, H0, jg, B, N, k, part)
        stats = [stats_of(part, 0)]
        acts = [None]
        mx = mn = amx = amn = abar = None
        for l in range(1, nb):
            Cin, Cout = widths[l - 1], widths[l]
            ldo = round_up(Cout, 4)
            last = l == nb - 1
            half = bool(last and training and aggr == 'max' and words is not None and nb >= 3 and
                        L.query('gpe_edge_lazy_dz3_ok', B, N, k, Cout, Cin) == 1 and (guard is None or guard.allow()))
            a = torch.empty(E, ldo, device=dev, dtype=torch.float16 if half else F32)
            part = torch.empty(nblk, 2, Cout, device=dev, dtype=torch.float64) if training else None
            agg = int(last and aggr == 'max')
            if agg:
                mx = torch.empty(BN, ldo, device=dev, dtype=F32)
                mn = torch.empty(BN, ldo, device=dev, dtype=F32)
                amx = torch.empty(BN, ldo, device=dev, dtype=torch.uint8)
                amn = torch.empty(BN, ldo, device=dev, dtype=torch.uint8)
            w_out = _word(words, l)
            wp, bf = pack_fold(Ws[l], params[4 * l + 1], stats[l - 1], ews if words is not None else None, ews_n, w_out)
            wr = 2 if words is not None else 0
            if l == 1:
                L.call('gpe_edge_mlp_fwd', 0, PQ, 2 * H0, jg, None, 0, B, N, k, Cin, Cout, wp, bf, a, ldo, part,
                       agg, mx, mn, amx, amn, ldo, _word(words, 0), w_out, ews, ews_n, wr)
            else:
                prev = acts[l - 1]
                L.call('gpe_edge_mlp_fwd', 1, None, 0, None, prev, prev.stride(0), B, N, k, Cin, Cout, wp, bf, a, ldo,
                       part, agg, mx, mn, amx, amn, ldo, _word(words, l - 1), w_out, ews, ews_n, int(half) | wr)
                if half and guard is not None and not guard.watch(w_out):
                    a = torch.empty(E, ldo, device=dev, dtype=F32)
                    L.call('gpe_edge_mlp_fwd', 1, None, 0, None, prev, prev.stride(0), B, N, k, Cin, Cout, wp, bf, a, ldo,
                           part, agg, mx, mn, amx, amn, ldo, _word(words, l - 1), w_out, ews, ews_n, 0)
            acts.append(a)
            stats.append(stats_of(part, l))
        Fo = widths[-1]
        ldF = round_up(Fo, 4)
        out = torch.empty(BN, ldF, device=dev, dtype=F32)[:, :Fo]
        if aggr == 'max':
            L.call('gpe_edge_finish', mx, mn, ldF, stats[-1], BN, Fo, out, ldF)
        else:
            abar = torch.empty(BN, ldF, device=dev, dtype=F32)
            L.call('gpe_edge_sum_k', acts[-1], ldF, BN, k, Fo, abar, ldF)
            L.call('gpe_scale', abar, 1.0 / k, abar, abar.numel())
            a_s, t_s = (1.0, 1.0) if aggr == 'mean' else (float(k), float(k))
            L.call('gpe_bn_apply_scaled', abar, ldF, stats[-1], BN, Fo, a_s, t_s, out, ldF)
        ctx.dims = (B, N, k, C, nb, aggr, training)
        ctx.widths = widths
        ctx.done = False
        ctx.words = words
        ctx.rev_job = None
        if fork and training:
            if order is None:
                del lane.jobs[:]
            ctx.rev_job = {'fn': knn_reverse, 'src': idx, 'out': None, 'event': None}
            lane.jobs.append(ctx.rev_job)
        ctx.save_for_backward(x, idx, jg, PQ, *params, *acts[1:], *stats,
                              *([mx, mn, amx, amn] if aggr == 'max' else [abar]))
        ctx.mark_non_differentiable(idx, order_out)
        return out, idx, order_out

    @staticmethod
    def backward(ctx, g_out, _g_idx, _g_order=None):
        if ctx.done:
            raise RuntimeError('EdgeConvFn.backward ran twice on the same graph: the stored activations are overwritten '
                               'in place by the first pass (retain_graph is not supported)')
        B, N, k, C, nb, aggr, training = ctx.dims
        if g_out is None:
            return (None,) * (11 + 4 * nb + 3 * nb)
        ctx.done = True
        widths = ctx.widths
        sv = ctx.saved_tensors
        x, idx, jg, PQ = sv[:4]
        params = sv[4: 4 + 4 * nb]
        acts = [None] + list(sv[4 + 4 * nb: 4 + 4 * nb + (nb - 1)])
        stats = list(sv[4 + 5 * nb - 1: 4 + 6 * nb - 1])
        tail = sv[4 + 6 * nb - 1:]
        Ws = [params[4 * l] for l in range(nb)]
        dev = x.device
        BN, E = B * N, B * N * k
        H0, Fo = widths[0], widths[-1]
        ldF = round_up(Fo, 4)
        if g_out.stride(1) != 1:
            g_out = g_out.contiguous()
        ldg = g_out.stride(0)
        grads = [None] * (4 * nb)
        words = ctx.words
        ews, ews_n = edge_workspace(B, N, k, max(ldF, 2 * H0), dev)
        rev, rev_event = None, None
        job = getattr(ctx, 'rev_job', None)
        lane = streams.lane(dev.index)
        if job is not None and job['out'] is not None:
            rev, rev_event = job['out'], job['event']
        elif SIDE_PQ and _side_ok(E):
            if job is not None and job in lane.jobs:
                lane.jobs.remove(job)
            with lane.fork([idx]):
                rev = knn_reverse(idx)

        psb = L.query('gpe_point_sums_blocks')
        part = torch.empty(psb, 2, Fo, device=dev, dtype=torch.float64)
        g_last, be_last = params[4 * (nb - 1) + 2], params[4 * (nb - 1) + 3]
        a_last = acts[-1]
        lz = (None, 0, None, None, 0, None)
        if aggr == 'max':
            mx, mn, amx, amn = tail
            lazy = a_last.dtype == torch.float16 and L.query('gpe_edge_lazy_dz3_ok', B, N, k, Fo, widths[-2]) == 1
            if a_last.dtype == torch.float16 and not lazy:
                a_last = a_last.float()
            L.call('gpe_edge_bwd_point_sums', g_out, ldg, mx, mn, ldF, stats[-1], BN, Fo, part,
                   _word(words, 2 * nb) if lazy else None)
            coef, dg, dbe = bn_bwd_coef(part, psb, stats[-1], Fo, E, g_last, be_last, training)
            if lazy:
                L.call('gpe_edge_dz3_bound', _word(words, 2 * nb), coef, Fo, _word(words, nb - 1), _word(words, 2 * nb - 1))
                lz = (g_out, ldg, amx, amn, ldF, coef)
            else:
                L.call('gpe_edge_dz3', a_last, ldF, g_out, ldg, amx, amn, ldF, coef, B, N, k, Fo, _word(words, 2 * nb - 1))
        else:
            abar, = tail
            gs = g_out
            if aggr == 'add':
                gs = torch.empty(BN, Fo, device=dev, dtype=F32)
                L.call('gpe_scale', g_out.contiguous(), float(k), gs, gs.numel())
            L.call('gpe_edge_bwd_point_sums', gs, gs.stride(0), abar, abar, ldF, stats[-1], BN, Fo, part, None)
            coef, dg, dbe = bn_bwd_coef(part, psb, stats[-1], Fo, E, g_last, be_last, training)
            L.call('gpe_edge_dz3_all', a_last, ldF, g_out, ldg, 1.0 / k if aggr == 'mean' else 1.0, coef, B, N, k, Fo,
                   _word(words, 2 * nb - 1))
        grads[4 * (nb - 1) + 2], grads[4 * (nb - 1) + 3] = _gret(g_last, dg), _gret(be_last, dbe)

        ws = torch.empty(max(L.query('gpe_redgemm_ws', widths[l], widths[l - 1]) for l in range(1, nb)), device=dev,
                         dtype=F32)
        dPQ = torch.empty(BN, 2 * H0, device=dev, dtype=F32)
        dz = a_last
        for l in range(nb - 1, 0, -1):
            Cl, Cp = widths[l], widths[l - 1]
            W, b = Ws[l], params[4 * l + 1]
            G = torch.empty(Cl, Cp, device=dev, dtype=F32)
            db = _gbuf(b)
            w_dz = _word(words, nb + l)
            if l == 1:
                L.call('gpe_edge_redgemm', dz, dz.stride(0), 0, None, 0, PQ, 2 * H0, jg, stats[0][0], B, N, k, Cl, Cp, G,
                       Cp, db, ws, w_dz, _word(words, 0), ews, ews_n, None, 0, None, None, 0, None)
            else:
                prev = acts[l - 1]
                L.call('gpe_edge_redgemm', dz, dz.stride(0), 1, prev, prev.stride(0), None, 0, None, stats[l - 1][0],
                       B, N, k, Cl, Cp, G, Cp, db, ws, w_dz, _word(words, l - 1), ews, ews_n,
                       *(lz if l == nb - 1 else (None, 0, None, None, 0, None)))
            sums = torch.empty(1, 2, Cp, device=dev, dtype=torch.float64)
            dW = _gbuf(W)
            L.call('gpe_bn_bwd_from_G', G, Cp, db, W, W.stride(0), Cl, Cp, stats[l - 1], sums, dW, Cp)
            gp, bp = params[4 * (l - 1) + 2], params[4 * (l - 1) + 3]
            coef_p, dgp, dbp = bn_bwd_coef(sums, 1, stats[l - 1], Cp, E, gp, bp, training)
            grads[4 * l], grads[4 * l + 1] = _gret(W, dW), _gret(b, db)
            grads[4 * (l - 1) + 2], grads[4 * (l - 1) + 3] = _gret(gp, dgp), _gret(bp, dbp)
            wt = pack_weight(W, transpose=True)
            if l == 1:
                dst = dz if dz.stride(0) == H0 else torch.empty(E, H0, device=dev, dtype=F32)
                L.call('gpe_edge_mlp_bwd', dz, dz.stride(0), 1, PQ, 2 * H0, jg, B, N, k, Cl, Cp, wt, coef_p, dst, H0,
                       dPQ, 2 * H0, w_dz, None, ews, ews_n, None, 0, None, None, 0, None)
                dz = dst
            else:
                prev = acts[l - 1]
                L.call('gpe_edge_mlp_bwd', dz, dz.stride(0), 0, None, 0, None, B, N, k, Cl, Cp, wt, coef_p, prev,
                       prev.stride(0), None, 0, w_dz, _word(words, nb + l - 1), ews, ews_n,
                       *(lz if l == nb - 1 else (None, 0, None, None, 0, None)))
                dz = prev

        if rev is not None:
            rev_off, rev_edge = rev
            lane.wait(made=rev, event=rev_event)
        else:
            rev_off, rev_edge = knn_reverse(idx)
        L.call('gpe_edge_pull_dq', dz, dz.stride(0), rev_off, rev_edge, B, N, k, H0, dPQ[:, H0:], 2 * H0)
        dWpq, dbpq = redgemm_raw(_rows2d(dPQ), _rows2d(x), BN, 2 * H0, C, want_colsum=True)
        W1, b1 = Ws[0], params[1]
        dW1 = _gbuf(W1)
        L.call('gpe_w1_grad_from_pq', dWpq, C, H0, C, dW1, 2 * C)
        db1 = _gbuf(b1)
        db1.copy_(dbpq[:H0])
        grads[0], grads[1] = _gret(W1, dW1), _gret(b1, db1)
        gx = None
        if ctx.needs_input_grad[0]:
            _, wpq_t, _ = edge_first_operands(W1, b1)
            gx = torch.empty(BN, C, device=dev, dtype=F32)
            linear_raw(_rows2d(dPQ), wpq_t, None, BN, C, 2 * H0, _rows2d(gx))
        return (gx, None, None, None, None, None, None, None, None, None, None, *grads, *([None] * (3 * nb)))


class EdgeInputsFn(torch.autograd.Function):

    @staticmethod
    def forward(ctx, x, idx, jg, B, N, k):
        _dev_check(x)
        C = x.shape[1]
        ld = round_up(2 * C, 4)
        out = torch.empty(B * N * k, ld, device=x.device, dtype=F32)
        L.call('gpe_edge_inputs_fwd', x, x.stride(0), C, jg, B * N, k, out, ld)
        ctx.save_for_backward(idx)
        ctx.dims = (B, N, k, C)
        return out[:, :2 * C]

    @staticmethod
    def backward(ctx, g):
        idx, = ctx.saved_tensors
        B, N, k, C = ctx.dims
        if g.stride(1) != 1:
            g = g.contiguous()
        rev_off, rev_edge = knn_reverse(idx)
        gx = torch.empty(B * N, C, device=g.device, dtype=F32)
        L.call('gpe_edge_inputs_bwd', g, g.stride(0), C, rev_off, rev_edge, B, N, k, gx, C)
        return gx, None, None, None, None, None


def edge_conv_general(x, B, N, k, training, eps, momentum, nb, aggr, tensors):
    idx, jg = knn(x, B, N, k, want_global=True)
    msg_in = EdgeInputsFn.apply(x, idx, jg, B, N, k)
    msg = DenseMLPFn.apply(msg_in, training, eps, momentum, nb, *tensors)
    if aggr == 'max':
        out = SegmentPoolFn.apply(msg, B * N, k, 1)
    elif aggr == 'add':
        out = SegmentPoolFn.apply(msg, B * N, k, 2)
    else:
        out = SegmentMeanFn.apply(msg, B * N, k)
    return out, idx


ASAP_K = 10
ASAP_F_MAX, ASAP_N_MAX = 512, 8192


def asap_count(N, ratio):
    if not ratio > 0:
        raise ValueError('pool ratio must be positive, got %r' % (ratio,))
    if ratio >= 1:
        return min(int(ratio), N)
    return int(math.ceil(np.float32(ratio) * np.float32(N)))


def asap_state_words(B, N, F, k):
    return 1024 + B * N * (2 * F + k + 8)


def asap_bwd_ws_bytes(B, N, F, k):
    nblk = min((B * N + 15) // 16, 1024)
    return 8 * (nblk + 1) * (5 * F + 3) + 4 * B * N * (F + k + 4)


class AsapPoolFn(torch.autograd.Function):

    @staticmethod
    def forward(ctx, x, B, N, ratio, order, save, trace, *params):
        _dev_check(x)
        F = x.shape[1]
        if not (1 <= F <= ASAP_F_MAX and 1 <= N <= ASAP_N_MAX) or x.shape[0] != B * N:
            raise ValueError('ASAP pooling takes 1 <= F <= %d features and 1 <= N <= %d points per cloud (got x %s for B=%d, '
                             'N=%d)' % (ASAP_F_MAX, ASAP_N_MAX, tuple(x.shape), B, N))
        k = min(ASAP_K, N)
        M = asap_count(N, ratio)
        xc = x if x.stride(1) == 1 else x.contiguous()
        idx = knn(xc, B, N, k, order=order)
        rev_off, rev_edge = knn_reverse(idx)
        dev = x.device
        state = torch.empty(asap_state_words(B, N, F, k), device=dev, dtype=F32)
        out = torch.empty(B * M, F, device=dev, dtype=F32)
        perm = torch.empty(B * M, device=dev, dtype=torch.int32)
        rank = torch.empty(B * N, device=dev, dtype=torch.int32)
        L.call('gpe_asap_fwd', xc, xc.stride(0), B, N, F, k, rev_off, rev_edge, *params, M, out, perm, rank, state)
        ctx.mark_non_differentiable(perm, rank, idx)
        ctx.dims = (B, N, F, k)
        if trace is not None:
            BN = B * N
            trace['winners'] = state[1024 + BN * F:1024 + 2 * BN * F].view(torch.int32).view(BN, F).clone()
            trace['fitness'] = state[1024 + BN * (2 * F + k + 6):1024 + BN * (2 * F + k + 7)].clone()
        if save:
            ctx.save_for_backward(xc, idx, rev_off, rev_edge, rank, state, *params)
        return out, perm, rank, idx

    @staticmethod
    def backward(ctx, gout, *_):
        xc, idx, rev_off, rev_edge, rank, state, *params = ctx.saved_tensors
        B, N, F, k = ctx.dims
        dev = xc.device
        gout = gout.contiguous()
        dx = torch.empty(B * N, F, device=dev, dtype=F32)
        grads = [_gbuf(p) for p in params]
        nws = asap_bwd_ws_bytes(B, N, F, k)
        L.call('gpe_asap_bwd', gout, xc, xc.stride(0), B, N, F, k, idx, rev_off, rev_edge, *params, rank, state, dx, F, *grads,
               _workspace(nws, dev))
        return (dx, None, None, None, None, None, None) + tuple(_gret(p, g) for p, g in zip(params, grads))


def asap_pool(x, B, N, params, ratio, order=None, trace=None):
    save = torch.is_grad_enabled() and (x.requires_grad or any(p.requires_grad for p in params))
    out, perm, rank, idx = AsapPoolFn.apply(x, B, N, ratio, order, save, trace, *params)
    if trace is not None:
        trace.update(perm=perm, rank=rank, knn=idx)
    return out, asap_count(N, ratio)


RNN_WS_HOOK = None


class RNNStackFn(torch.autograd.Function):

    @staticmethod
    def forward(ctx, x, h0, c0, T, n_layers, kind, want_state, h0_ok, *params):
        _dev_check(x)
        streams.lane(x.device.index).run_jobs()
        ctx.set_materialize_grads(False)
        dev = x.device
        lstm = kind == 'lstm'
        G = 4 if lstm else 3
        seq = x.dim() == 3
        Bn, In = x.shape[0], x.shape[-1]
        Hh = h0.shape[2]
        Hp = round_up(Hh, 4)
        Lr = n_layers
        hs = torch.zeros(Lr, Bn, T + 1, Hp, device=dev, dtype=F32)
        hs[:, :, 0, :Hh].copy_(h0)
        cs = None
        if lstm:
            cs = torch.empty(Lr, T + 1, Bn, Hh, device=dev, dtype=F32)
            cs[:, 0].copy_(c0)
        saved = torch.empty(Lr, T, Bn, 4 * Hh, device=dev, dtype=F32)
        w_ih0, _, b_ih0, b_hh0 = params[0:4]
        bias0 = bias_sum(b_ih0, b_hh0) if lstm else gru_bias(b_ih0, b_hh0, Hh)
        if seq:
            xproj = torch.empty(Bn, T, G * Hh, device=dev, dtype=F32)
            linear_raw(_rows3d(x), pack_weight(w_ih0), bias0, Bn * T, G * Hh, In, (xproj, G * Hh, 0, 0))
            xp_sb, xp_st = T * G * Hh, G * Hh
        else:
            xproj = torch.empty(Bn, G * Hh, device=dev, dtype=F32)
            linear_raw(_rows2d(x), pack_weight(w_ih0), bias0, Bn, G * Hh, In, _rows2d(xproj))
            xp_sb, xp_st = G * Hh, 0
        whh, wih, biases, bhns = [], [None], [None], []
        for l in range(Lr):
            w_ih, w_hh, b_ih, b_hh = params[4 * l: 4 * l + 4]
            whh.append(pack_gates(w_hh, Hh, G))
            if l > 0:
                wih.append(pack_gates(w_ih, Hh, G))
                biases.append(bias_sum(b_ih, b_hh) if lstm else gru_bias(b_ih, b_hh, Hh))
            bhns.append(None if lstm else b_hh[2 * Hh:])
        pl_hh, am_hh, pl_ih, am_ih = [], [], [None], [None]
        for l in range(Lr):
            w_ih, w_hh = params[4 * l], params[4 * l + 1]
            a, b = planned_planes(w_hh, K_GATES_H3)
            pl_hh.append(a); am_hh.append(b)
            if l > 0:
                a, b = planned_planes(w_ih, K_GATES_H3)
                pl_ih.append(a); am_ih.append(b)
        h3 = bool(h0_ok) and all(t is not None for t in pl_hh + am_hh + pl_ih[1:] + am_ih[1:])
        keep = (whh, wih, biases, pl_hh, am_hh, pl_ih, am_ih)
        ws_n = L.query('gpe_rnn_seq_fwd_ws', G, Lr, T, Bn, Hh)
        ws = torch.empty(ws_n, device=dev, dtype=torch.uint8) if ws_n > 0 else None
        if RNN_WS_HOOK is not None:
            RNN_WS_HOOK('fwd', ws)
        L.call('gpe_rnn_seq_fwd', G, Lr, T, Bn, Hh, xproj, xp_sb, xp_st, _ptr_array(whh), _ptr_array(wih),
               _ptr_array(biases), None if lstm else _ptr_array(bhns), hs, hs.stride(0), hs.stride(1), hs.stride(2),
               cs, cs.stride(0) if lstm else 0, cs.stride(1) if lstm else 0, saved, saved.stride(0), saved.stride(1),
               _ptr_array(pl_hh) if h3 else None, _ptr_array(pl_ih) if h3 else None,
               _ptr_array(am_hh) if h3 else None, _ptr_array(am_ih) if h3 else None, ws, max(ws_n, 0))
        del keep
        hN = cN = None
        if want_state:
            hN = hs[:, :, T, :Hh].contiguous()
            cN = cs[:, T].contiguous() if lstm else None
        ctx.dims = (Bn, In, Hh, T, Lr, kind, seq)
        ctx.save_for_backward(x, hs, cs, saved, *params)
        ctx.needs_state_grad = (h0.requires_grad, c0 is not None and c0.requires_grad)
        top = hs[Lr - 1, :, 1:, :Hh]
        if lstm:
            return top, hN, cN
        return top, hN

    @staticmethod
    def backward(ctx, g_top, g_hN, g_cN=None):
        Bn, In, Hh, T, Lr, kind, seq = ctx.dims
        lstm = kind == 'lstm'
        G = 4 if lstm else 3
        sv = ctx.saved_tensors
        x, hs, cs, saved = sv[:4]
        params = sv[4:]
        dev = x.device
        want_h0, want_c0 = ctx.needs_state_grad
        GH = G * Hh
        GHp = round_up(GH, 4)
        dgx = torch.empty(Lr, Bn, T, GHp, device=dev, dtype=F32)
        dgh = dgx if lstm else torch.empty(Lr, Bn, T, GHp, device=dev, dtype=F32)
        part = torch.empty(L.query('gpe_rnn_seq_bwd_ws', G, Lr, T, Bn, Hh), device=dev, dtype=F32)
        if RNN_WS_HOOK is not None:
            RNN_WS_HOOK('bwd', part)
        carry = torch.empty(2, Lr, Bn, Hh, device=dev, dtype=F32)
        whh_t = [pack_weight(params[4 * l + 1], transpose=True) for l in range(Lr)]
        wih_t = [None] + [pack_weight(params[4 * l], transpose=True) for l in range(1, Lr)]
        if g_top is not None and g_top.stride(2) != 1:
            g_top = g_top.contiguous()
        ghN = g_hN.contiguous() if g_hN is not None else None
        gcN = g_cN.contiguous() if (lstm and g_cN is not None) else None
        tp_hh, ta_hh, tp_ih, ta_ih = [], [], [None], [None]
        if lstm:
            for l in range(Lr):
                a, b = planned_planes(params[4 * l + 1], K_TRANS_H3)
                tp_hh.append(a); ta_hh.append(b)
                if l > 0:
                    a, b = planned_planes(params[4 * l], K_TRANS_H3)
                    tp_ih.append(a); ta_ih.append(b)
        h3b = lstm and all(t is not None for t in tp_hh + ta_hh + tp_ih[1:] + ta_ih[1:])
        L.call('gpe_rnn_seq_bwd', G, Lr, T, Bn, Hh, g_top, g_top.stride(0) if g_top is not None else 0,
               g_top.stride(1) if g_top is not None else 0, ghN, gcN, _ptr_array(whh_t), _ptr_array(wih_t),
               hs, hs.stride(0), hs.stride(1), hs.stride(2), cs, cs.stride(0) if lstm else 0, cs.stride(1) if lstm else 0,
               saved, saved.stride(0), saved.stride(1), dgx, dgh, dgx.stride(0), dgx.stride(1), dgx.stride(2), part, carry,
               _ptr_array(tp_hh) if h3b else None, _ptr_array(tp_ih) if h3b else None,
               _ptr_array(ta_hh) if h3b else None, _ptr_array(ta_ih) if h3b else None)
        grads = [None] * (4 * Lr)
        d_x = None
        d_h0 = torch.empty(Lr, Bn, Hh, device=dev, dtype=F32) if want_h0 else None
        d_c0 = carry[0].clone() if want_c0 else None
        nz = (GH + 255) // 256
        dGs = None
        gx0 = _rows3d(dgx[0][:, :, :GH])
        if not seq:
            dGs = torch.empty(Bn, GH, device=dev, dtype=F32)
            L.call('gpe_reduce_inner', dgx[0], T * GHp, GHp, T, Bn, GH, dGs, GH, 0)
            if ctx.needs_input_grad[0]:
                d_x = torch.empty(Bn, In, device=dev, dtype=F32)
                linear_raw(_rows2d(dGs), pack_weight(params[0], transpose=True), None, Bn, In, GH, _rows2d(d_x))
        elif ctx.needs_input_grad[0]:
            d_x = torch.empty(Bn, T, In, device=dev, dtype=F32)
            linear_raw(gx0, pack_weight(params[0], transpose=True), None, Bn * T, In, GH, (d_x, In, 0, 0))
        if want_h0:
            for l in range(Lr):
                rec = torch.empty(nz, Bn, Hh, device=dev, dtype=F32)
                L.call('gpe_linear_splitk', dgh[l][:, 0], T * GHp, whh_t[l], rec, Bn, Hh, GH)
                L.call('gpe_reduce_inner', rec, Hh, Bn * Hh, nz, Bn, Hh, d_h0[l], Hh, 0)
                if not lstm:
                    L.call('gpe_add', d_h0[l], carry[0][l], d_h0[l], Bn * Hh)
        with side_grads(list(params), [dgx, dgh, hs, x, dGs]):
            for l in range(Lr):
                w_ih, w_hh, b_ih, b_hh = params[4 * l: 4 * l + 4]
                gx_rows, gh_rows = _rows3d(dgx[l][:, :, :GH]), _rows3d(dgh[l][:, :, :GH])
                d_whh, d_bhh = _gbuf(w_hh), _gbuf(b_hh)
                redgemm_raw(gh_rows, _rows3d(hs[l][:, :T, :Hh]), Bn * T, GH, Hh, out=(d_whh, d_bhh))
                d_wih, d_bih = _gbuf(w_ih), _gbuf(b_ih)
                if l == 0 and not seq:
                    redgemm_raw(_rows2d(dGs), _rows2d(x), Bn, GH, In, out=(d_wih, d_bih))
                else:
                    Kin = In if l == 0 else Hh
                    src = _rows3d(x) if l == 0 else _rows3d(hs[l - 1][:, 1:, :Hh])
                    redgemm_raw(gx_rows, src, Bn * T, GH, Kin, out=(d_wih, d_bih))
                grads[4 * l: 4 * l + 4] = [_gret(w_ih, d_wih), _gret(w_hh, d_whh), _gret(b_ih, d_bih),
                                           _gret(b_hh, d_bhh)]
        return (d_x, d_h0, d_c0, None, None, None, None, None, *grads)


class DropoutMulFn(torch.autograd.Function):

    @staticmethod
    def forward(ctx, x, mask):
        _dev_check(x)
        assert x.dim() == 3 and x.stride(2) == 1 and mask.is_contiguous() and mask.shape == x.shape
        Bn, T, H = x.shape
        out = torch.empty(Bn, T, H, device=x.device, dtype=F32)
        L.call('gpe_mul_rows', x, x.stride(0), x.stride(1), mask, Bn, T, H, out)
        ctx.save_for_backward(mask)
        return out

    @staticmethod
    def backward(ctx, g):
        mask, = ctx.saved_tensors
        if g.stride(2) != 1:
# ... 931 lines not shown
```

include/gpe_hip.h:

```cpp
#ifndef GPE_HIP_H
#define GPE_HIP_H
#include <stdint.h>
#ifdef __cplusplus
extern "C" {
#endif

int gpe_abi_version(void);
int gpe_debug_set(int flags);
int gpe_debug_get(void);
int gpe_reserve_cus_set(int n);
int gpe_math_set(int mode);
int gpe_math_get(void);
long gpe_f16x3_min_rows(void);
long gpe_f16x3_min_rows_set(long rows);

long gpe_knn_ws_bytes(int B, int N, int C, int k);
int gpe_knn(const float* x, int B, int N, int C, int ldx, int k, int32_t* idx, int32_t* idx_glob, const int32_t* order_in,
            int32_t* order_out, void* ws, long ws_bytes, void* stream);

int gpe_knn_reverse(const int32_t* idx, int B, int N, int k, int32_t* rev_off, int32_t* rev_edge, void* stream);

long gpe_packed_size(int N, int K);
int gpe_pack_weight(const float* w, int ldw, int N, int K, int transpose, const float* col_scale,
                    float* wp, void* stream);
long gpe_packed_planes_size(int Npad, int K);
long gpe_pack_job_blocks(int kind, long total, int Npad, int K);
int gpe_pack_multi(const void* jobs_dev, int njobs, long total_blocks, void* stream);
int gpe_pack_fold(const float* w, int ldw, int N, int K, const float* col_scale, const float* t, const float* bias, float* wp,
                  float* bias_out, void* ws, long ws_bytes, uint32_t* clear_word, uint32_t* ticket, void* stream);
int gpe_fold_bias(const float* w, int ldw, int N, int K, const float* bias, const float* t, float* out,
                  void* stream);

int gpe_linear(const float* a, long a_so, long a_si, int a_inner,
               const float* wp, const float* bias,
               const float* addend, long ad_so, long ad_si, int ad_inner,
               float* y, long y_so, long y_si, int y_inner,
               int M, int N, int K, int act, void* stream);

long gpe_redgemm_ws(int Mg, int Ng);
int gpe_redgemm(const float* u, long u_so, long u_si, int u_inner,
                const float* v, long v_so, long v_si, int v_inner, const float* v_shift,
                long rows, int Mg, int Ng, float* G, int ldg, float* colsum, float* part, int accumulate,
                void* stream);


int gpe_stats_blocks(void);
int gpe_edge_gather_stats(const float* pq, int ldpq, int H, const int32_t* jg, int B, int N, int k,
                          double* part, void* stream);

int gpe_bn_finalize(const double* part, int nblk, int C, double count, const float* gamma, const float* beta,
                    float eps, float momentum, float* running_mean, float* running_var, int64_t* num_batches,
                    float* stats_out, void* stream);
int gpe_bn_from_running(const float* running_mean, const float* running_var, int C, const float* gamma,
                        const float* beta, float eps, float* stats_out, void* stream);

int gpe_edge_mlp_fwd(int a_mode, const float* pq, int ldpq, const int32_t* jg, const float* a_in, int lda,
                     int B, int N, int k, int Cin, int Cout, const float* wp, const float* bias,
                     float* out, int ldo, double* stats_part,
                     int agg, float* mx, float* mn, uint8_t* amx, uint8_t* amn, int ldagg,
                     const uint32_t* amax_a, uint32_t* amax_out, void* ws, long ws_bytes, int out_half, void* stream);
long gpe_edge_ws_bytes(int B, int N, int k, int ldmax);
int gpe_edge_pq_amax(const float* pq, int ldpq, int H, long rows, uint32_t* amax, void* ws, long ws_bytes, void* stream);
int gpe_absmax(const float* x, int ldx, long rows, int cols, uint32_t* amax, void* stream);

int gpe_edge_finish(const float* mx, const float* mn, int ldagg, const float* stats, long rows, int C,
                    float* y, int ldy, void* stream);

int gpe_point_sums_blocks(void);
int gpe_edge_bwd_point_sums(const float* g, int ldg, const float* mx, const float* mn, int ldagg,
                            const float* stats, long rows, int C, double* part, uint32_t* amax_sg, void* stream);
int gpe_bn_bwd_coef(const double* part, int nblk, const float* stats, int C, double count, float* coef,
                    float* dgamma, float* dbeta, void* stream);
int gpe_bn_bwd_from_G(const float* G, int ldG, const float* db, const float* w_next, int ldw, int Cn, int C,
                      const float* stats, double* sums, float* dw, int lddw, void* stream);

int gpe_edge_dz3(float* a3, int lda3, const float* g, int ldg, const uint8_t* amx, const uint8_t* amn, int ldagg,
                 const float* coef, int B, int N, int k, int F, uint32_t* amax_out, void* stream);

int gpe_edge_redgemm(const float* u, int ldu, int v_mode, const float* v, int ldv, const float* pq, int ldpq,
                     const int32_t* jg, const float* v_shift, int B, int N, int k, int Mg, int Ng, float* G, int ldG,
                     float* colsum, float* part, const uint32_t* amax_u, const uint32_t* amax_v, void* ws, long ws_bytes,
                     const float* lz_g, int lz_ldg, const uint8_t* lz_amx, const uint8_t* lz_amn, int lz_ldagg,
                     const float* lz_coef, void* stream);

int gpe_edge_mlp_bwd(const float* a, int lda, int act_mode, const float* pq, int ldpq, const int32_t* jg,
                     int B, int N, int k, int Cin, int Cout, const float* wp, const float* coef_out,
                     float* dz_out, int ldo, float* dP, int lddp, const uint32_t* amax_a, uint32_t* amax_out, void* ws,
                     long ws_bytes, const float* lz_g, int lz_ldg, const uint8_t* lz_amx, const uint8_t* lz_amn, int lz_ldagg,
                     const float* lz_coef, void* stream);
int gpe_edge_lazy_dz3_ok(int B, int N, int k, int F, int Cprev);
int gpe_edge_dz3_bound(const uint32_t* amax_sg, const float* coef, int F, const uint32_t* amax_a3, uint32_t* amax_out, void* stream);

int gpe_edge_pull_dq(const float* dz, int lddz, const int32_t* rev_off, const int32_t* rev_edge,
                     int B, int N, int k, int H, float* dQ, int lddq, void* stream);

int gpe_segment_mean_fwd(const float* x, int ldx, int B, int N, int C, float* y, int ldy, void* stream);
int gpe_segment_mean_bwd(const float* gy, int ldgy, int B, int N, int C, float* gx, int ldgx, int accumulate,
                         void* stream);

int gpe_lstm_cell_fwd(float* gates, const float* c_prev, long ldc_prev, float* c, float* h, long h_stride,
                      int Bn, int H, void* stream);
int gpe_lstm_cell_bwd(const float* dh_out, long dho_stride, const float* dh_rec, int n_rec, const float* dc_next,
                      const float* gates, const float* c, const float* c_prev, long ldc_prev,
                      float* dgates, long dg_stride, float* dc_prev, int Bn, int H, void* stream);

long gpe_packed_gates_size(int H, int K);
int gpe_pack_weight_gates(const float* w, int ldw, int H, int K, float* wp, void* stream);
int gpe_lstm_step_fwd(const float* h_prev, long hp_stride, const float* whh_gates_packed, const float* xproj,
                      long xp_stride, const float* c_prev, long ldc_prev, float* gates, float* c_out, float* h_out,
                      long h_stride, int Bn, int H, void* stream);

long gpe_packed_ngates_size(int H, int G, int K);
int gpe_pack_weight_ngates(const float* w, int ldw, int H, int G, int K, float* wp, void* stream);
int gpe_gru_step_fwd(const float* h_prev, long hp_stride, const float* whh_gates_packed, const float* xproj,
                     long xp_stride, const float* bhn, float* saved, float* h_out, long h_stride, int Bn, int H,
                     void* stream);
int gpe_gru_cell_bwd(const float* dh_out, long dho_stride, const float* dh_rec, int n_rec, const float* dh_dir_next,
                     const float* saved, const float* h_prev, long hp_stride, float* dgx, float* dgh, long dg_stride,
                     float* dh_dir_prev, int Bn, int H, void* stream);

int gpe_rnn_seq_fwd(int gates, int L, int T, int Bn, int H, const float* xproj0, long xp0_sb, long xp0_st,
                    const void* const* whh, const void* const* wih, const void* const* bias, const void* const* bhn,
                    float* hs, long hs_sl, long hs_sb, long hs_st, float* cs, long cs_sl, long cs_st, float* saved,
                    long sv_sl, long sv_st, const void* const* whh_pl, const void* const* wih_pl,
                    const void* const* whh_amax, const void* const* wih_amax, void* ws, long ws_bytes, void* stream);
long gpe_rnn_seq_fwd_ws(int gates, int L, int T, int Bn, int H);
long gpe_rnn_seq_bwd_ws(int gates, int L, int T, int Bn, int H);
int gpe_rnn_seq_bwd(int gates, int L, int T, int Bn, int H, const float* dtop, long dt_sb, long dt_st, const float* d_hN,
                    const float* d_cN, const void* const* whh_t, const void* const* wih_t, const float* hs, long hs_sl,
                    long hs_sb, long hs_st, const float* cs, long cs_sl, long cs_st, const float* saved, long sv_sl,
                    long sv_st, float* dgx, float* dgh, long dg_sl, long dg_sb, long dg_st, float* part, float* carry,
                    const void* const* whh_tpl, const void* const* wih_tpl, const void* const* whh_amax,
                    const void* const* wih_amax, void* stream);

int gpe_sparsemax_fwd(const float* z, int ldz, long rows, int W, float* out, int ldo, void* stream);
int gpe_sparsemax_bwd(const float* out, int ldo, const float* g, int ldg, long rows, int W, float* gz, int ldgz,
                      void* stream);
int gpe_sparsemax_loss(const float* x, int ldx, const int32_t* target, long rows, int W, float* gx, int ldg, double* part,
                       float* loss, int* bad, void* stream);
int gpe_bn_apply(const float* a, int lda, const float* stats, long rows, int C, float* y, int ldy, void* stream);

int gpe_bn_apply_scaled(const float* a, int lda, const float* stats, long rows, int C, float a_scale, float t_scale,
                        float* y, int ldy, void* stream);
int gpe_edge_sum_k(const float* a, int lda, long npts, int k, int F, float* out, int ldo, void* stream);
int gpe_edge_inputs_fwd(const float* x, int ldx, int C, const int32_t* jg, long npts, int k, float* out, int ldo,
                        void* stream);
int gpe_edge_inputs_bwd(const float* g, int ldg, int C, const int32_t* rev_off, const int32_t* rev_edge, int B, int N, int k,
                        float* gx, int ldgx, void* stream);
int gpe_edge_dz3_all(float* a3, int lda3, const float* g, int ldg, float gscale, const float* coef, int B, int N, int k,
                     int F, uint32_t* amax_out, void* stream);

int gpe_segment_pool_fwd(const float* x, int ldx, int B, int N, int C, int mode, float* y, int ldy, int32_t* arg,
                         void* stream);
int gpe_segment_pool_bwd(const float* gy, int ldgy, const int32_t* arg, int B, int N, int C, int mode, float* gx,
                         int ldgx, void* stream);

long gpe_attn_pool_ws(int B, int N, int P, int C);
int gpe_attn_pool_fwd(const float* w, int ldw, const float* feat, int ldf, int B, int N, int P, int C, int mode,
                      float* out, int32_t* arg, float* part, int32_t* part_arg, void* stream);
int gpe_attn_pool_bwd(const float* w, int ldw, const float* feat, int ldf, const float* g, const int32_t* arg, int B,
                      int N, int P, int C, int mode, float* gw, int ldgw, float* gf, int ldgf, void* stream);

int gpe_fps(const float* pos, int ldp, int B, int N, int C, int M, const int32_t* start, int32_t* idx, void* stream);
int gpe_radius(const float* pos, int ldp, const int32_t* cidx, int B, int N, int C, int M, float r, int maxn,
               int32_t* nbr, int32_t* cnt, void* stream);
int gpe_pointconv_self_loops(const int32_t* nbr, const int32_t* cnt, int B, int N, int M, int maxn, int32_t* cnt_out,
                             int32_t* drop, void* stream);
int gpe_ball_messages(const float* pos, int ldp, const float* x, int ldx, int Cx, const int32_t* cidx, const int32_t* nbr,
                      const int64_t* off, const int32_t* drop, int B, int N, int C, int M, int maxn, float* msg, int ldm,
                      int32_t* seg_of_row, void* stream);
int gpe_ragged_max_fwd(const float* x, int ldx, const int64_t* off, long S, int C, float* y, int ldy, int64_t* arg,
                       void* stream);
int gpe_ragged_max_bwd(const float* gy, int ldgy, const int64_t* off, const int64_t* arg, const int32_t* seg_of_row, long E,
                       int C, float* gx, int ldgx, void* stream);

int gpe_pattern_loss_fwd(const float* ol, long ol_sb, long ol_sp, long ol_sl, const float* rot, long rot_s,
                         const float* tr, long tr_s, const float* gt_ol, const float* gt_rot, const float* gt_tr,
                         const int32_t* num_edges, int B, int P, int L, int R, int T, int flags, float pad0, float pad1,
                         float loop_w, double* part, float* loop_sums, float* out5, void* stream);
int gpe_pattern_loss_bwd(const float* ol, long ol_sb, long ol_sp, long ol_sl, const float* rot, long rot_s,
                         const float* tr, long tr_s, const float* gt_ol, const float* gt_rot, const float* gt_tr,
                         const int32_t* num_edges, int B, int P, int L, int R, int T, int flags, float pad0, float pad1,
                         float loop_w, const float* loop_sums, const float* gscale, float* g_ol, float* g_rot,
                         float* g_tr, void* stream);
int gpe_origin_match(const float* ol, long ol_sb, long ol_sp, long ol_sl, const float* gt_ol, int D,
                     const int32_t* num_edges, int B, int P, int L, float* gt_out, int32_t* lead, void* stream);
int gpe_order_match(const float* pred_feat, const float* gt_feat, int B, int P, int D, int64_t* perm, int32_t* fail,
                    void* stream);

int gpe_stitch_loss_fwd(const float* tags, long t_sb, long t_sp, long t_sl, int D, const float* logit, long m_sb, long m_sp,
                        long m_sl, const int64_t* stitches, const int64_t* nums, int S, const float* gt_mask,
                        const float* gt_tags, int B, int P, int L, int flags, float margin, float sup_w, double* part,
                        float* out5, void* stream);
int gpe_stitch_loss_bwd(const float* tags, long t_sb, long t_sp, long t_sl, int D, const float* logit, long m_sb, long m_sp,
                        long m_sl, const int64_t* stitches, const int64_t* nums, int S, const float* gt_mask,
                        const float* gt_tags, int B, int P, int L, int flags, float margin, float sup_w, const double* part,
                        const float* gscale, float* g_tags, float* g_mask, void* stream);
int gpe_stitch_renumber(const int64_t* stitches, const int64_t* nums, int B, int S, int P, int L, const int64_t* perm,
                        const int32_t* lead, const int32_t* num_edges, int64_t* out, void* stream);
int gpe_panel_shift(const float* feat, int D, const int32_t* lead, const int32_t* num_edges, long npanels, int L, float* out,
                    void* stream);

int gpe_quality_panels(const float* ol, long ol_sb, long ol_sp, long ol_sl, const float* gt_ol, const int32_t* num_edges,
                       const int32_t* num_panels, const float* rot, long rot_s, const float* gt_rot, int R, const float* tr,
                       long tr_s, const float* gt_tr, int T, int B, int P, int L, int flags, const float* stats_host,
                       double* part, void* stream);
int gpe_quality_stitches(const float* tags, long t_sb, long t_sp, long t_sl, int D, const float* logit, long m_sb, long m_sp,
                         long m_sl, const int64_t* stitches, const int64_t* nums, int S, const float* gt_mask, int B, int P,
                         int L, int flags, const float* stats_host, double* part, void* stream);
int gpe_quality_finalize(const double* part, int B, int P, int L, int flags, float* out, int32_t* counts, void* stream);

int gpe_asap_fwd(const float* x, int ldx, int B, int N, int F, int k, const int32_t* rev_off, const int32_t* rev_edge,
                 const float* w_lin, const float* b_lin, const float* w_att, const float* b_att, const float* w1, const float* b1,
                 const float* w2, const float* w3, const float* b3, int M, float* out, int32_t* perm, int32_t* rank, float* state,
                 void* stream);
int gpe_asap_bwd(const float* dout, const float* x, int ldx, int B, int N, int F, int k, const int32_t* idx, const int32_t* rev_off,
                 const int32_t* rev_edge, const float* w_lin, const float* b_lin, const float* w_att, const float* b_att,
                 const float* w1, const float* b1, const float* w2, const float* w3, const float* b3, const int32_t* rank,
                 const float* state, float* dx, int lddx, float* g_wlin, float* g_blin, float* g_watt, float* g_batt, float* g_w1,
                 float* g_b1, float* g_w2, float* g_w3, float* g_b3, void* ws, void* stream);

int gpe_stitch_pairs_pack(const float* w, int ldw, int N, int K, const float* col_scale, float* out, int ldo, void* stream);
int gpe_stitch_pairs_planes(const float* wt, int K, int ldw, const uint32_t* amax, void* out, void* stream);
int gpe_stitch_pairs_fwd(const float* ab, int ldab, int H, int n_layers, const float* wpk, const void* planes,
                         const uint32_t* w_amax, const float* last_stats, const int32_t* num_edges, int B, int P, int L,
                         uint64_t* table, float* logits, void* stream);
int gpe_stitch_pairs_rows(const float* edges3d, const int32_t* num_edges, int B, int P, int L, int Fe, const float* shift_host,
                          const float* scale_host, int c0, int c1, long rows_chunk, float* rows, void* stream);
int gpe_stitch_pairs_reduce(const float* y, long ldy, const int32_t* num_edges, int B, int P, int L, int c0, int c1,
                            long rows_chunk, uint64_t* table, float* logits, void* stream);
int gpe_stitch_select(const uint64_t* table, int B, int P, int L, int32_t* stitches, int32_t* num_stitches, float* scores,
                      void* stream);

int gpe_stitch_pairs_labels(const int32_t* gt_stitches, const int32_t* gt_num_stitches, int B, int P, int L, int S, uint32_t* mask,
                            void* stream);
int gpe_stitch_pairs_eval_fwd(const float* ab, int ldab, int H, int n_layers, const float* wpk, const void* planes,
                              const uint32_t* w_amax, const float* last_stats, const int32_t* num_edges, int B, int P, int L,
                              uint64_t* table, float* logits, const uint32_t* mask, double* loss_slab, uint64_t* counters,
                              void* stream);
int gpe_stitch_pairs_eval_reduce(const float* y, long ldy, const int32_t* num_edges, int B, int P, int L, int c0, int c1,
                                 long rows_chunk, uint64_t* table, float* logits, const uint32_t* mask, double* loss_slab,
                                 uint64_t* counters, void* stream);
int gpe_stitch_eval_finalize(const double* loss_slab, long slots, int group, const uint64_t* counters, const uint32_t* mask,
                             const int32_t* stitches, const int32_t* num_stitches, int B, int P, int L, double* loss_sum,
                             int32_t* counts, float* metrics, void* stream);

int gpe_pair_loss_fwd(const float* x, const void* y, int kind, long M, int slots, void* part, uint32_t* ticket, float* out,
                      int32_t* counts, void* stream);
int gpe_pair_loss_bwd(const float* x, const void* y, int kind, long M, const float* gscale, float* gx, void* stream);

int gpe_stitch_sample(const float* edges3d, const int32_t* num_edges, const int32_t* gt_stitches, const int32_t* gt_num_stitches,
                      int G, int P, int L, int Fe, int S, const int32_t* index, int B, int n_stitched, int n_non_stitched,
                      int flags , const float* shift_host, const float* scale_host,
                      uint64_t* state , uint32_t* ticket, float* rows, uint8_t* labels, int32_t* status,
                      void* stream);


int gpe_mesh_points_sample(const float* verts4, const int32_t* faces, const int32_t* vert_off, const int32_t* face_off,
                           const uint32_t* face_cdf, int G, const int32_t* index, int B, int N, float point_noise_w,
                           const float* shift_host, const float* scale_host, int relabel, float* ws,
                           uint64_t* state , uint32_t* ticket, float* features, int64_t* segmentation,
                           int32_t* status, void* stream);

int gpe_adam_step(float* p, float* g, float* m, float* v, long n, float lr, float beta1, float beta2, float eps,
                  float weight_decay, long step, float gscale, int zero_grad, void* stream);
int gpe_adam_step_dev(float* p, float* g, float* m, float* v, long n, const float* hyper, float beta1, float beta2, float eps,
                      float weight_decay, float gscale, int zero_grad, void* stream);
int gpe_adam_hyper(float lr, float beta1, float beta2, long step, float* out_host);
int gpe_standardize(const float* x, long rows, int C, const float* shift_host, const float* scale_host, float* out,
                    void* stream);

int gpe_linear_splitk(const float* a, long a_so, const float* wp, float* y, int M, int N, int K, void* stream);

int gpe_reduce_inner(const float* x, long x_so, long x_si, int T, int R, int C, float* y, int ldy,
                     int accumulate, void* stream);
int gpe_w1_grad_from_pq(const float* dwpq, int ld, int H, int C, float* dw1, int lddw1, void* stream);
int gpe_w1_split(const float* w1, int ldw1, const float* b1, int H, int C, float* wpq, int ldwpq, float* bias_pq,
                 void* stream);
int gpe_scale(const float* x, float alpha, float* out, long n, void* stream);
int gpe_scale_dev(const float* x, const float* alpha, float* out, long n, void* stream);
int gpe_add(const float* a, const float* b, float* out, long n, void* stream);
int gpe_mul_rows(const float* x, long x_sb, long x_st, const float* mask, long Bn, int T, int H, float* out, void* stream);

#ifdef __cplusplus
}
#endif
#endif
```

Baseline: 3672 garments/s.

## Fuse first EdgeConv layer weight-gradient reduction into B2 backward GEMM epilogue

```diff
diff --git a/garment-pattern-estimation_amd/csrc/gpe_edge_dispatch.h b/garment-pattern-estimation_amd/csrc/gpe_edge_dispatch.h
--- a/garment-pattern-estimation_amd/csrc/gpe_edge_dispatch.h
+++ b/garment-pattern-estimation_amd/csrc/gpe_edge_dispatch.h
@@ -30,6 +30,9 @@
 int gpe_edge_f16x3_scales(RgParams& p, long npts, int amode, int emode, int KCH, hipStream_t s);
 int gpe_edge_f16x3(const RgParams& p, int amode, int emode, int NT, int KCH, int stats_nblk, hipStream_t s);
 int gpe_edge_w8(const RgParams& p, int amode, int emode, int NT, int KCH, int stats_nblk, hipStream_t s);
+int gpe_edge_w8_enabled(int kind);
+
+bool gpe_edge_first_ok(int B, int N, int k, int C, int H0, int H1);
 
 template <int A, int E> struct GpeEdgeMode { static constexpr int amode = A, emode = E, kind = gpe_edge_kind(A, E); };
 template <int AQ_, int BQ_, int KCH_> struct GpeEdgeTile { static constexpr int AQ = AQ_, BQ = BQ_, KCH = KCH_, NT = 4 * AQ_ + BQ_; };
@@ -62,12 +65,17 @@
 
 #define GPE_EDGE_LDS_CAP (160 * 1024)
 #define GPE_EDGE_LDS_CAP_STATIC (160 * 1024 - 64)
+static inline int gpe_edge_grid(int num_tiles, int stats_nblk)
+{
+    int gx = gpe_num_cus();
+    if (gx > num_tiles) gx = num_tiles;
+    if (stats_nblk > 0 && gx > stats_nblk) gx = stats_nblk;
+    return gx;
+}
 template <auto KERNEL, int BLOCK, int LDS_CAP> static int gpe_edge_launch(const RgParams& p, int stats_nblk, size_t lds, hipStream_t s)
 {
     GPE_ENSURE_MAX_LDS_N(KERNEL, LDS_CAP);
-    int gx = gpe_num_cus();
-    if (gx > p.num_tiles) gx = p.num_tiles;
-    if (stats_nblk > 0 && gx > stats_nblk) gx = stats_nblk;
+    const int gx = gpe_edge_grid(p.num_tiles, stats_nblk);
     hipLaunchKernelGGL(KERNEL, dim3(gx), dim3(BLOCK), lds, s, p, stats_nblk);
     GPE_CHECK_LAUNCH();
     return GPE_EDGE_LAUNCHED;
diff --git a/garment-pattern-estimation_amd/csrc/gpe_edge_dispatch.hip b/garment-pattern-estimation_amd/csrc/gpe_edge_dispatch.hip
--- a/garment-pattern-estimation_amd/csrc/gpe_edge_dispatch.hip
+++ b/garment-pattern-estimation_amd/csrc/gpe_edge_dispatch.hip
@@ -74,10 +74,19 @@
     return rc == GPE_OK ? GPE_EDGE_LAUNCHED : rc;
 }
 
+bool gpe_edge_first_ok(int B, int N, int k, int C, int H0, int H1)
+{
+    if (g_eg_math != 3 || k != 16 || B <= 0 || N <= 0 || C < 1 || C > 4) return false;
+    if (!gpe_edge_width_ok(H0) || !gpe_edge_width_ok(H1) || (H0 & 3)) return false;
+    if (gpe_edge_chunks(H0) != 13 || gpe_edge_chunks(H1) != 13 || 2 * ((H1 + 3) & ~3) < 384) return false;
+    const long rows = (long)B * N * k;
+    return rows >= gpe_h3_min_rows() && rows < (1L << 31) && gpe_edge_w8_enabled(GPE_EDGE_B2) != 0;
+}
+
 int gpe_edgegemm_try(const RgParams& p, int amode, int emode, int stats_nblk, hipStream_t s)
 {
     const int math = g_eg_math;
-    const bool f16_only = p.out_half || p.lz_g;
+    const bool f16_only = p.out_half || p.lz_g || p.fr_part;
     if (!gpe_edge_on_menu(p, amode, emode)) return f16_only ? GPE_EINVAL : GPE_EDGE_NOT_MINE;
     const int NT = gpe_edge_chunks(p.N), KCH = gpe_edge_chunks(p.K);
 
@@ -95,6 +104,7 @@
         rc = gpe_edge_f16x3_scales(q, p.M / p.k, amode, emode, KCH, s);
         if (rc != GPE_OK) return rc;
         rc = gpe_edge_w8(q, amode, emode, NT, KCH, stats_nblk, s);
+        if (rc == GPE_EDGE_NOT_MINE && p.fr_part) return GPE_EINVAL;
         if (rc == GPE_EDGE_NOT_MINE) rc = gpe_edge_f16x3(q, amode, emode, NT, KCH, stats_nblk, s);
         rc = gpe_edge_finish(rc, q, fold, s);
         if (rc == GPE_EDGE_LAUNCHED && q.amax_out && p.tracked) *p.tracked = 1;
diff --git a/garment-pattern-estimation_amd/csrc/gpe_edgegemm_w8.hip b/garment-pattern-estimation_amd/csrc/gpe_edgegemm_w8.hip
--- a/garment-pattern-estimation_amd/csrc/gpe_edgegemm_w8.hip
+++ b/garment-pattern-estimation_amd/csrc/gpe_edgegemm_w8.hip
@@ -17,6 +17,7 @@
     }
     return tab[kind];
 }
+int gpe_edge_w8_enabled(int kind) { return w8_enabled(kind); }
 
 int gpe_edge_w8(const RgParams& p, int amode, int emode, int NT, int KCH, int stats_nblk, hipStream_t s)
 {
@@ -26,6 +27,7 @@
     if (kbytes < (KCH == 13 ? 384 : 256)) return GPE_EDGE_NOT_MINE;
     if (p.out_half && !(p.k == 16 && emode == E_EDGE_FWD && amode == A_DENSE && p.agg)) return GPE_EINVAL;
     if (p.lz_g && !(p.k == 16 && emode == E_BWD_INPLACE && amode == A_DENSE)) return GPE_EINVAL;
+    if (p.fr_part && !(p.k == 16 && emode == E_BWD_GATHER)) return GPE_EINVAL;
     if (!w8_enabled(gpe_edge_kind(amode, emode))) return GPE_EDGE_NOT_MINE;
     return p.k == 16 ? w8_select<16>(p, amode, emode, NT, KCH, stats_nblk, s)
            : p.k == 5 ? gpe_w8_select_k5(p, amode, emode, NT, KCH, stats_nblk, s)
diff --git a/garment-pattern-estimation_amd/csrc/gpe_edgegemm_w8_b2r.hip b/garment-pattern-estimation_amd/csrc/gpe_edgegemm_w8_b2r.hip
--- /dev/null
+++ b/garment-pattern-estimation_amd/csrc/gpe_edgegemm_w8_b2r.hip
@@ -0,0 +1,13 @@
+#define W8_SLOT_FENCE 1
+#include "gpe_edgegemm_w8_kernel.h"
+
+int gpe_w8_launch_b2_first(const RgParams& p, int stats_nblk, hipStream_t s)
+{
+    if (!p.fr_x || !p.fr_part || p.fr_C < 1 || p.fr_C > 4 || p.fr_ld < p.N || (p.fr_ld & 3)) return GPE_EINVAL;
+    switch (p.fr_C) {
+    case 1: return w8_launch<13, 13, A_DENSE, E_BWD_GATHER, -1, false, 16, 1>(p, stats_nblk, s);
+    case 2: return w8_launch<13, 13, A_DENSE, E_BWD_GATHER, -1, false, 16, 2>(p, stats_nblk, s);
+    case 3: return w8_launch<13, 13, A_DENSE, E_BWD_GATHER, -1, false, 16, 3>(p, stats_nblk, s);
+    default: return w8_launch<13, 13, A_DENSE, E_BWD_GATHER, -1, false, 16, 4>(p, stats_nblk, s);
+    }
+}
diff --git a/garment-pattern-estimation_amd/csrc/gpe_edgegemm_w8_kernel.h b/garment-pattern-estimation_amd/csrc/gpe_edgegemm_w8_kernel.h
--- a/garment-pattern-estimation_amd/csrc/gpe_edgegemm_w8_kernel.h
+++ b/garment-pattern-estimation_amd/csrc/gpe_edgegemm_w8_kernel.h
@@ -8,15 +8,19 @@
 #ifndef W8_B2_SC1
 #define W8_B2_SC1 1
 #endif
+#ifndef W8_FRED_RING
+#define W8_FRED_RING 3
+#endif
 #ifndef W8_BUFSTORE
 #define W8_BUFSTORE 11
 #endif
 __device__ __forceinline__ void w8_pin4(float4& v) { asm volatile("" : "+v"(v.x), "+v"(v.y), "+v"(v.z), "+v"(v.w)); }
 
-template <int NT, int KCH, int AMODE, int EMODE, int AGGT, bool LAZY, int KK = 16>
+template <int NT, int KCH, int AMODE, int EMODE, int AGGT, bool LAZY, int KK = 16, int FRED = 0>
 __global__ __launch_bounds__(512) void gpe_edgegemm_w8_kernel(RgParams p, int stats_nblk)
 {
     using SP = SplitF16x2;
+    static_assert(FRED == 0 || (EMODE == E_BWD_GATHER && KK == 16 && NT == 13 && KCH == 13 && FRED <= 4), "first-block reduction: the B2 instance");
     static_assert(KK == 16 || KK == 5 || KK == 4, "neighbourhood sizes with a compile-time row schedule");
     static_assert(!LAZY || KK == 16, "lazy dz3 needs one point per wave");
     constexpr int NPW = 16 / KK;
@@ -48,7 +52,7 @@
     constexpr int I1 = C0 + 4;
     constexpr int C1 = (NSLOT >= 28) ? 22 : 16;
     constexpr int EP0 = NSLOT - 16;
-    constexpr int RING = (GATHER_ACT && NPW > 1) ? 6 : 8;
+    constexpr int RING = (GATHER_ACT && NPW > 1) ? 6 : FRED ? W8_FRED_RING : 8;
 
     extern __shared__ __align__(16) float smem[];
     __shared__ unsigned amax_sh[4];
@@ -127,11 +131,13 @@
     int vz;
     asm volatile("v_mov_b32 %0, 0" : "=v"(vz));
     int rbl = rb;
+    int fsl = (int)blockIdx.x * 4 + pt;
 #define W8_REFRESH_SCALARS()                                   \
     {                                                          \
         int sz_;                                               \
         asm volatile("s_mov_b32 %0, 0" : "=s"(sz_));           \
         rbl = rb + sz_;                                        \
+        fsl = (int)blockIdx.x * 4 + pt + sz_;                  \
     }
     auto load_jgv = [&](int tile) -> int {
         const long row0 = (long)tile * TR;
@@ -210,6 +216,40 @@
         __amdgpu_buffer_rsrc_t orsrc = __builtin_amdgcn_make_buffer_rsrc(p.out, 0, 0, 0x00020000);
         float amax_t = 0.f;
         int jgv_e = 0, jgv_cur = 0;
+        constexpr int FC = FRED ? FRED : 1;
+        float fx_cur[FC];
+        float4 fq[FC], fl[2] = {zero4, zero4};
+#pragma unroll
+        for (int d = 0; d < FC; ++d) { fx_cur[d] = 0.f; fq[d] = zero4; }
+        constexpr int FNCH = 2 * FRED + 1;
+        auto frow = [&](int i) -> float* { return p.fr_part + ((long)fsl * FNCH + i) * p.fr_ld + (unsigned)cn; };
+        if constexpr (ROLE == 1 && FRED > 0) {
+#pragma unroll
+            for (int i = 0; i < FNCH; ++i) st4(frow(i), zero4);
+        }
+        auto flush_load = [&](int i) { fl[i & 1] = ld4(frow(i)); };
+        auto flush_add = [&](int i) {
+            float4 a = fl[i & 1];
+            if (i < FRED) {
+                const float xi = __int_as_float(__builtin_amdgcn_readlane(__float_as_int(fx_cur[i < FRED ? i : 0]), RW));
+                a.x = __builtin_fmaf(dp.x, xi, a.x); a.y = __builtin_fmaf(dp.y, xi, a.y);
+                a.z = __builtin_fmaf(dp.z, xi, a.z); a.w = __builtin_fmaf(dp.w, xi, a.w);
+            } else {
+                const float4 b = i < 2 * FRED ? fq[i < 2 * FRED ? i - FRED : 0] : dp;
+                a.x += b.x; a.y += b.y; a.z += b.z; a.w += b.w;
+            }
+            st4(frow(i), a);
+        };
+        auto issue_x_loads = [&](int tile_x, int jv) {
+            if constexpr (FRED > 0) {
+                const long npts = p.M / KK;
+                long pi = (long)tile_x * 4 + pt;
+                pi = pi < npts - 1 ? pi : npts - 1;
+                const float* xr = p.fr_x + ((lane < RW) ? (long)jv : pi) * p.fr_ldx;
+#pragma unroll
+                for (int d = 0; d < FRED; ++d) fx_cur[d] = xr[d];
+            }
+        };
 
         auto issue_stage_loads = [&](int tile_s, int h) {
             const long row0 = (long)tile_s * TR;
@@ -316,10 +356,11 @@
             e_rv = (int)((p.M - e_row0 < TR) ? (p.M - e_row0) : TR);
             epi_on = on && rbl < e_rv;
             constexpr int ES = OUTH ? 2 : 4;
-            orsrc = __builtin_amdgcn_make_buffer_rsrc(reinterpret_cast<char*>(p.out) + e_row0 * p.ldo * ES, 0, RG_BM * p.ldo * ES, 0x00020000);
+            if constexpr (FRED == 0)
+                orsrc = __builtin_amdgcn_make_buffer_rsrc(reinterpret_cast<char*>(p.out) + e_row0 * p.ldo * ES, 0, RG_BM * p.ldo * ES, 0x00020000);
 #pragma unroll
             for (int t = 0; t < 4; ++t) { s32[t] = 0.f; q32[t] = 0.f; vmx[t] = -INFINITY; vmn[t] = INFINITY; imx[t] = 0; imn[t] = 0; }
-            dp = zero4;
+            if constexpr (FRED == 0) dp = zero4;
             amax_t = 0.f;
             if constexpr (GATHER_ACT) {
                 const long ptl = (long)tile_e * (4 * NPW) + (e_rv - 1) / KK;
@@ -387,11 +428,20 @@
                 o.y = (av.y > 0.f) ? __builtin_fmaf(z.y, cs4.y, __builtin_fmaf(k24.y, av.y, c14.y)) : 0.f;
                 o.z = (av.z > 0.f) ? __builtin_fmaf(z.z, cs4.z, __builtin_fmaf(k24.z, av.z, c14.z)) : 0.f;
                 o.w = (av.w > 0.f) ? __builtin_fmaf(z.w, cs4.w, __builtin_fmaf(k24.w, av.w, c14.w)) : 0.f;
+                if constexpr (FRED > 0) {
+#pragma unroll
+                    for (int d = 0; d < FRED; ++d) {
+                        const float xs = __int_as_float(__builtin_amdgcn_readlane(__float_as_int(fx_cur[d]), u));
+                        fq[d].x = __builtin_fmaf(o.x, xs, fq[d].x); fq[d].y = __builtin_fmaf(o.y, xs, fq[d].y);
+                        fq[d].z = __builtin_fmaf(o.z, xs, fq[d].z); fq[d].w = __builtin_fmaf(o.w, xs, fq[d].w);
+                    }
+                } else {
                 const gpe_u32x4 oq = {__float_as_uint(o.x), __float_as_uint(o.y), __float_as_uint(o.z), __float_as_uint(o.w)};
                 if constexpr ((W8_BUFSTORE & (EMODE == E_BWD_INPLACE ? 4 : 8)) != 0)
                     __builtin_amdgcn_raw_buffer_store_b128(oq, orsrc, cn * 4, r * p.ldo * 4, (GATHER_ACT && W8_B2_SC1) ? 16 : 0);
                 else
                     st4(p.out + (e_row0 + r) * p.ldo + cn, o);
+                }
                 if constexpr (EMODE == E_BWD_INPLACE)
                     amax_t = fmaxf(fmaxf(amax_t, fmaxf(fabsf(o.x), fabsf(o.y))), fmaxf(fabsf(o.z), fabsf(o.w)));
                 dp.x += o.x; dp.y += o.y; dp.z += o.z; dp.w += o.w;
@@ -407,7 +457,7 @@
                         *reinterpret_cast<uchar4*>(p.oamx + o) = make_uchar4(imx[0], imx[1], imx[2], imx[3]);
                         *reinterpret_cast<uchar4*>(p.oamn + o) = make_uchar4(imn[0], imn[1], imn[2], imn[3]);
                     }
-                    if constexpr (GATHER_ACT) st4(p.dP + gpt * p.lddp + cn, dp);
+                    if constexpr (GATHER_ACT && FRED == 0) st4(p.dP + gpt * p.lddp + cn, dp);
                 }
                 amax_run = fmaxf(amax_run, amax_t);
                 if constexpr (FWD) {
@@ -491,6 +541,17 @@
                             begin_epi(tile_e, do_epi);
                             if constexpr (GATHER_ACT) { jgv_cur = jgv_e; jgv_e = load_jgv(tile); }
                         }
+                        if constexpr (FRED > 0) {
+                            static_assert(FNCH + 2 <= EP0, "the additions end before the epilogue starts");
+                            if (q >= 2 && q - 2 < FNCH) flush_add(q - 2);
+                            if (q < FNCH) flush_load(q);
+                            if (q == FRED + 2) issue_x_loads(tile_e, jgv_cur);
+                            if (q == FNCH + 1) {
+                                dp = zero4;
+#pragma unroll
+                                for (int d = 0; d < FRED; ++d) fq[d] = zero4;
+                            }
+                        }
                         if (q >= EP0 && q - EP0 < RW) {
                             epi_row(q - EP0, zq);
                             if (q - EP0 + RING < RW) issue_act_load(q - EP0 + RING, tile_e, jgv_cur);
@@ -586,11 +647,23 @@
                 W8_REFRESH_SCALARS()
                 begin_epi(prev >= 0 ? prev : 0, prev >= 0);
                 jgv_cur = jgv_e;
+                if constexpr (FRED > 0) {
+#pragma unroll
+                    for (int i = 0; i < FNCH; ++i) { flush_load(i); flush_add(i); }
+                    dp = zero4;
+#pragma unroll
+                    for (int d = 0; d < FRED; ++d) fq[d] = zero4;
+                    issue_x_loads(prev >= 0 ? prev : 0, jgv_cur);
+                }
 #pragma unroll
                 for (int u = 0; u < RW; ++u) {
                     epi_row(u, ld4(&Cs[(rbl + u) * LDC + cn]));
                     if (u + RING < RW) issue_act_load(u + RING, prev >= 0 ? prev : 0, jgv_cur);
                 }
+            }
+            if constexpr (FRED > 0) {
+#pragma unroll
+                for (int i = 0; i < FNCH; ++i) { flush_load(i); flush_add(i); }
             }
             if (p.amax_out && !GATHER_ACT) {
                 float m = amax_run;
@@ -638,13 +711,13 @@
 #undef W8_REFRESH_SCALARS
 }
 
-template <int NT, int KCH, int AMODE, int EMODE, int AGGT, bool LAZY, int KK = 16>
+template <int NT, int KCH, int AMODE, int EMODE, int AGGT, bool LAZY, int KK = 16, int FRED = 0>
 static int w8_launch(const RgParams& p, int stats_nblk, hipStream_t s)
 {
     constexpr int LDC = 16 * NT + 4;
     constexpr int AWORDS = (2 * RG_BM * 16 * x6_pchunks(KCH)) / 4;
     const size_t lds = (size_t)(2 * AWORDS + RG_BM * LDC) * sizeof(float);
-    return gpe_edge_launch<gpe_edgegemm_w8_kernel<NT, KCH, AMODE, EMODE, AGGT, LAZY, KK>, 512, GPE_EDGE_LDS_CAP_STATIC>(p, stats_nblk, lds, s);
+    return gpe_edge_launch<gpe_edgegemm_w8_kernel<NT, KCH, AMODE, EMODE, AGGT, LAZY, KK, FRED>, 512, GPE_EDGE_LDS_CAP_STATIC>(p, stats_nblk, lds, s);
 }
 
 struct W8Menu {
@@ -656,6 +729,7 @@
 };
 int gpe_w8_launch_f3(const RgParams& p, int stats_nblk, hipStream_t s);
 int gpe_w8_launch_b3(const RgParams& p, int stats_nblk, hipStream_t s);
+int gpe_w8_launch_b2_first(const RgParams& p, int stats_nblk, hipStream_t s);
 
 template <int KK>
 static int w8_select(const RgParams& p, int amode, int emode, int NT, int KCH, int stats_nblk, hipStream_t s)
@@ -666,6 +740,9 @@
         if ((M::kind == GPE_EDGE_F2 && p.agg) || (M::kind == GPE_EDGE_F3 && !p.agg)) return GPE_EDGE_NOT_MINE;
         if constexpr (KK == 16 && M::kind == GPE_EDGE_F3) return gpe_w8_launch_f3(p, stats_nblk, s);
         else if constexpr (KK == 16 && M::kind == GPE_EDGE_B3) return gpe_w8_launch_b3(p, stats_nblk, s);
-        else return w8_launch<T::NT, T::KCH, M::amode, M::emode, M::kind == GPE_EDGE_F2 ? 0 : M::kind == GPE_EDGE_F3 ? 1 : -1, false, KK>(p, stats_nblk, s);
+        else if constexpr (KK == 16 && M::kind == GPE_EDGE_B2) {
+            if (p.fr_part) return gpe_w8_launch_b2_first(p, stats_nblk, s);
+            return w8_launch<T::NT, T::KCH, M::amode, M::emode, -1, false, KK>(p, stats_nblk, s);
+        } else return w8_launch<T::NT, T::KCH, M::amode, M::emode, M::kind == GPE_EDGE_F2 ? 0 : M::kind == GPE_EDGE_F3 ? 1 : -1, false, KK>(p, stats_nblk, s);
     });
 }
diff --git a/garment-pattern-estimation_amd/csrc/gpe_rowgemm.h b/garment-pattern-estimation_amd/csrc/gpe_rowgemm.h
--- a/garment-pattern-estimation_amd/csrc/gpe_rowgemm.h
+++ b/garment-pattern-estimation_amd/csrc/gpe_rowgemm.h
@@ -39,6 +39,8 @@
     const uint8_t* lz_amx; const uint8_t* lz_amn; int lz_ldagg;
     const float* lz_coef;
     int out_half;
+    const float* fr_x; int fr_ldx; int fr_C;
+    float* fr_part; int fr_ld;
     int w_ready;
     const unsigned* user_amax_a;
     unsigned* user_amax_out;
diff --git a/garment-pattern-estimation_amd/csrc/gpe_rowgemm.hip b/garment-pattern-estimation_amd/csrc/gpe_rowgemm.hip
--- a/garment-pattern-estimation_amd/csrc/gpe_rowgemm.hip
+++ b/garment-pattern-estimation_amd/csrc/gpe_rowgemm.hip
@@ -469,3 +469,91 @@
     if (rc == GPE_OK && amax_out && !tracked) rc = gpe_h3_absmax(amax_out, dz_out, p.M, Cout, ldo, s);
     return rc;
 }
+
+extern "C" int gpe_edge_first_reduce_ok(int B, int N, int k, int C, int H0, int H1, const void* reserved)
+{
+    (void)reserved;
+    return gpe_edge_first_ok(B, N, k, C, H0, H1) ? 1 : 0;
+}
+static long edge_first_slots(int B, int N, int k) { return 4L * gpe_edge_grid(gpe_cdiv((long)B * N * k, RG_BM), 0); }
+extern "C" int gpe_edge_first_part_floats(int B, int N, int k, int C, int H0, const void* reserved)
+{
+    (void)reserved;
+    if (B <= 0 || N <= 0 || k != 16 || C < 1 || C > 4 || H0 <= 0 || (H0 & 3) || (long)B * N * k >= (1L << 31)) return GPE_EINVAL;
+    return (int)(edge_first_slots(B, N, k) * (2 * C + 1) * H0);
+}
+extern "C" int gpe_edge_mlp_bwd_first(const float* a, int lda, const float* pq, int ldpq, const int32_t* jg, int B, int N, int k,
+                                      int Cin, int Cout, const float* wp, const float* coef_out, const uint32_t* amax_a, void* ws,
+                                      long ws_bytes, const float* x, int ldx, int C, float* part, long part_floats, void* stream)
+{
+    if (!a || !wp || !coef_out || !pq || !jg || !x || !part || B <= 0 || N <= 0 || lda < Cin || (ldpq & 3) || ldpq < 2 * Cout ||
+        ldx < C || !gpe_edge_first_ok(B, N, k, C, Cout, Cin))
+        return GPE_EINVAL;
+    if (part_floats < edge_first_slots(B, N, k) * (2 * C + 1) * Cout || (((uintptr_t)part) & 15)) return GPE_EINVAL;
+    {
+        const size_t E_ = (size_t)B * N * k, P_ = (size_t)B * N, pb = (size_t)part_floats * 4;
+        if (gpe_overlap(part, pb, a, E_ * lda * 4) || gpe_overlap(part, pb, pq, P_ * ldpq * 4) || gpe_overlap(part, pb, x, P_ * ldx * 4))
+            return GPE_EINVAL;
+    }
+    RgParams p = {};
+    p.M = (long)B * N * k; p.N = Cout; p.K = Cin;
+    p.R = (RG_BM / k) * k; p.num_tiles = gpe_cdiv(p.M, p.R);
+    p.a = GpeRows{a, lda, 0, 0};
+    p.pq = pq; p.ldpq = ldpq; p.H = Cout; p.jg = jg; p.k = k; p.rcp_k = 1.0 / k;
+    p.wp = wp; p.Npad = gpe_round_up(Cout, 16);
+    p.coef_out = coef_out;
+    p.fr_x = x; p.fr_ldx = ldx; p.fr_C = C; p.fr_part = part; p.fr_ld = Cout;
+    p.dbg = g_gpe_dbg; p.pin_clouds = B;
+    p.user_amax_a = amax_a; p.ws = gpe_edge_ws(ws, ws_bytes);
+    p.rev = gpe_walk_rev(1);
+    int tracked = 0;
+    p.tracked = &tracked;
+    const int rc = gpe_edgegemm_try(p, A_DENSE, E_BWD_GATHER, 0, (hipStream_t)stream);
+    return rc == 1 ? GPE_OK : (rc < 0 ? rc : GPE_EINVAL);
+}
+
+#define EF_RUNS 32
+#define EF_COLS 32
+__global__ __launch_bounds__(EF_COLS * EF_RUNS) void gpe_edge_first_finish_kernel(const float* __restrict__ part, long slots, int C, int H0,
+                                                                              float* __restrict__ dw1, int lddw1, float* __restrict__ db1)
+{
+    __shared__ double red[2][EF_RUNS][EF_COLS];
+    const int lane = threadIdx.x % EF_COLS, run = threadIdx.x / EF_COLS;
+    const int c = blockIdx.x * EF_COLS + lane, d = blockIdx.y;
+    const long per = (slots + EF_RUNS - 1) / EF_RUNS, s0 = run * per, s1 = (s0 + per < slots) ? s0 + per : slots;
+    const long slot_f = (long)(2 * C + 1) * H0;
+    const int r0 = d < C ? d : 2 * C, r1 = d < C ? C + d : 2 * C;
+    double a0 = 0.0, a1 = 0.0;
+    if (c < H0) {
+        const float* sl = part + s0 * slot_f + c;
+        long s = s0;
+        for (; s + 16 <= s1; s += 16, sl += 16 * slot_f) {
+            float v0[16], v1[16];
+#pragma unroll
+            for (int t = 0; t < 16; ++t) { v0[t] = sl[t * slot_f + (long)r0 * H0]; v1[t] = sl[t * slot_f + (long)r1 * H0]; }
+#pragma unroll
+            for (int t = 0; t < 16; ++t) { a0 += (double)v0[t]; a1 += (double)v1[t]; }
+        }
+        for (; s < s1; ++s, sl += slot_f) { a0 += (double)sl[(long)r0 * H0]; a1 += (double)sl[(long)r1 * H0]; }
+    }
+    red[0][run][lane] = a0; red[1][run][lane] = a1;
+    __syncthreads();
+    if (run == 0 && c < H0) {
+        double p0 = 0.0, q0 = 0.0;
+        for (int r = 0; r < EF_RUNS; ++r) { p0 += red[0][r][lane]; q0 += red[1][r][lane]; }
+        if (d < C) {
+            dw1[(size_t)c * lddw1 + d] = (float)p0;
+            dw1[(size_t)c * lddw1 + C + d] = (float)(q0 - p0);
+        } else
+            db1[c] = (float)p0;
+    }
+}
+extern "C" int gpe_edge_first_finish(const float* part, int B, int N, int k, int C, int H0, float* dw1, int lddw1, float* db1,
+                                     void* stream)
+{
+    if (!part || !dw1 || !db1 || B <= 0 || N <= 0 || k != 16 || C < 1 || C > 4 || H0 <= 0 || (H0 & 3) || lddw1 < 2 * C) return GPE_EINVAL;
+    hipLaunchKernelGGL(gpe_edge_first_finish_kernel, dim3(gpe_cdiv(H0, EF_COLS), C + 1), dim3(EF_COLS * EF_RUNS), 0, (hipStream_t)stream, part,
+                       edge_first_slots(B, N, k), C, H0, dw1, lddw1, db1);
+    GPE_CHECK_LAUNCH();
+    return GPE_OK;
+}
diff --git a/garment-pattern-estimation_amd/ops.py b/garment-pattern-estimation_amd/ops.py
--- a/garment-pattern-estimation_amd/ops.py
+++ b/garment-pattern-estimation_amd/ops.py
@@ -91,6 +91,7 @@
 
 
 SIDE_GRADS = not (os.environ.get('GPE_DEBUG') == '1' and os.environ.get('GPE_SIDE_GRADS') == '0')
+FIRST_BLOCK_REDUCE = True
 SIDE_MIN_EDGES = 1 << 17
 SIDE_PQ = not (os.environ.get('GPE_DEBUG') == '1' and os.environ.get('GPE_SIDE_PQ') == '0')
 _LAST_EDGES = [0]
@@ -624,6 +625,11 @@
         return True
 
 
+def _first_reduce_ok(needs_x_grad, x, B, N, k, C, H0, H1):
+    return bool(FIRST_BLOCK_REDUCE and not needs_x_grad and x.stride(1) == 1 and
+                L.query('gpe_edge_first_reduce_ok', B, N, k, C, H0, H1, None) == 1)
+
+
 class EdgeConvFn(torch.autograd.Function):
 
     @staticmethod
@@ -727,8 +733,9 @@
         if fork and training:
             if order is None:
                 del lane.jobs[:]
-            ctx.rev_job = {'fn': knn_reverse, 'src': idx, 'out': None, 'event': None}
-            lane.jobs.append(ctx.rev_job)
+            if not _first_reduce_ok(ctx.needs_input_grad[0], x, B, N, k, C, H0, widths[1]):
+                ctx.rev_job = {'fn': knn_reverse, 'src': idx, 'out': None, 'event': None}
+                lane.jobs.append(ctx.rev_job)
         ctx.save_for_backward(x, idx, jg, PQ, *params, *acts[1:], *stats,
                               *([mx, mn, amx, amn] if aggr == 'max' else [abar]))
         ctx.mark_non_differentiable(idx, order_out)
@@ -764,7 +771,11 @@
         rev, rev_event = None, None
         job = getattr(ctx, 'rev_job', None)
         lane = streams.lane(dev.index)
-        if job is not None and job['out'] is not None:
+        first_reduce = _first_reduce_ok(ctx.needs_input_grad[0], x, B, N, k, C, H0, widths[1])
+        if first_reduce:
+            if job is not None and job in lane.jobs:
+                lane.jobs.remove(job)
+        elif job is not None and job['out'] is not None:
             rev, rev_event = job['out'], job['event']
         elif SIDE_PQ and _side_ok(E):
             if job is not None and job in lane.jobs:
@@ -804,7 +815,7 @@
 
         ws = torch.empty(max(L.query('gpe_redgemm_ws', widths[l], widths[l - 1]) for l in range(1, nb)), device=dev,
                          dtype=F32)
-        dPQ = torch.empty(BN, 2 * H0, device=dev, dtype=F32)
+        dPQ = None if first_reduce else torch.empty(BN, 2 * H0, device=dev, dtype=F32)
         dz = a_last
         for l in range(nb - 1, 0, -1):
             Cl, Cp = widths[l], widths[l - 1]
@@ -828,7 +839,15 @@
             grads[4 * l], grads[4 * l + 1] = _gret(W, dW), _gret(b, db)
             grads[4 * (l - 1) + 2], grads[4 * (l - 1) + 3] = _gret(gp, dgp), _gret(bp, dbp)
             wt = pack_weight(W, transpose=True)
-            if l == 1:
+            if l == 1 and first_reduce:
+                W1, b1 = Ws[0], params[1]
+                part = torch.empty(L.query('gpe_edge_first_part_floats', B, N, k, C, H0, None), device=dev, dtype=F32)
+                L.call('gpe_edge_mlp_bwd_first', dz, dz.stride(0), PQ, 2 * H0, jg, B, N, k, Cl, Cp, wt, coef_p, w_dz, ews, ews_n,
+                       x, x.stride(0), C, part, part.numel())
+                dW1, db1 = _gbuf(W1), _gbuf(b1)
+                L.call('gpe_edge_first_finish', part, B, N, k, C, H0, dW1, 2 * C, db1)
+                grads[0], grads[1] = _gret(W1, dW1), _gret(b1, db1)
+            elif l == 1:
                 dst = dz if dz.stride(0) == H0 else torch.empty(E, H0, device=dev, dtype=F32)
                 L.call('gpe_edge_mlp_bwd', dz, dz.stride(0), 1, PQ, 2 * H0, jg, B, N, k, Cl, Cp, wt, coef_p, dst, H0,
                        dPQ, 2 * H0, w_dz, None, ews, ews_n, None, 0, None, None, 0, None)
@@ -840,6 +859,8 @@
                        *(lz if l == nb - 1 else (None, 0, None, None, 0, None)))
                 dz = prev
 
+        if first_reduce:
+            return (None, None, None, None, None, None, None, None, None, None, None, *grads, *([None] * (3 * nb)))
         if rev is not None:
             rev_off, rev_edge = rev
             lane.wait(made=rev, event=rev_event)
diff --git a/include/gpe_hip.h b/include/gpe_hip.h
--- a/include/gpe_hip.h
+++ b/include/gpe_hip.h
@@ -90,6 +90,14 @@
                      const float* lz_coef, void* stream);
 int gpe_edge_lazy_dz3_ok(int B, int N, int k, int F, int Cprev);
 int gpe_edge_dz3_bound(const uint32_t* amax_sg, const float* coef, int F, const uint32_t* amax_a3, uint32_t* amax_out, void* stream);
+
+int gpe_edge_first_reduce_ok(int B, int N, int k, int C, int H0, int H1, const void* reserved);
+int gpe_edge_first_part_floats(int B, int N, int k, int C, int H0, const void* reserved);
+int gpe_edge_mlp_bwd_first(const float* a, int lda, const float* pq, int ldpq, const int32_t* jg, int B, int N, int k,
+                           int Cin, int Cout, const float* wp, const float* coef_out, const uint32_t* amax_a, void* ws,
+                           long ws_bytes, const float* x, int ldx, int C, float* part, long part_floats, void* stream);
+int gpe_edge_first_finish(const float* part, int B, int N, int k, int C, int H0, float* dw1, int lddw1, float* db1,
+                          void* stream);
 
 int gpe_edge_pull_dq(const float* dz, int lddz, const int32_t* rev_off, const int32_t* rev_edge,
                      int B, int N, int k, int H, float* dQ, int lddq, void* stream);
```

Result: faster. 3746 garments/s (median of 4 runs) (+2.0%).
